# littlepure2333/GFlow

Measured on AMD Instinct MI355X. Metric: GFlow fit_video frames/sec (fwd+bwd+step) @60k Gaussians 480p, higher is better.
Workload: dtype f32

## Files before the change

gflow_amd/_lib.py:

```python
import ctypes
import os
import subprocess
import threading

import torch

_HERE = os.path.dirname(os.path.abspath(__file__))
_CSRC = os.path.join(_HERE, "csrc")
LIB_PATH = os.environ.get("GFLOW_HIP_LIB") or os.path.join(_HERE, "libgflow_hip.so")

_lock = threading.Lock()
_lib = None

c_void_p, c_int, c_float, c_size_t, c_int64 = ctypes.c_void_p, ctypes.c_int, ctypes.c_float, ctypes.c_size_t, ctypes.c_int64

MIN_VERSION = 308

_P = c_void_p
SIGNATURES = {
    "gfl_version": (c_int, []),
    "gfl_constants": (c_int, [_P]),
    "gfl_constants_n": (c_int, [_P, c_int]),
    "gfl_ewa_on_mfma": (c_int, []),
    "gfl_status_string": (ctypes.c_char_p, [c_int]),
    "gfl_last_hip_error": (c_int, []),
    "gfl_reduce_workspace_bytes": (c_size_t, [c_int]),
    "gfl_project_point_fwd": (c_int, [_P, _P, _P, c_int, c_int, c_int, c_float, c_float, _P, _P, _P]),
    "gfl_project_point_bwd": (c_int, [_P, _P, _P, _P, _P, _P, c_int, _P, _P, _P, c_size_t, _P]),
    "gfl_cov3d_fwd": (c_int, [_P, _P, _P, c_int, _P, _P]),
    "gfl_cov3d_bwd": (c_int, [_P, _P, _P, _P, c_int, _P, _P, _P]),
    "gfl_ewa_fwd": (c_int, [_P, _P, _P, _P, _P, _P, c_int, c_int, c_int, _P, _P, _P, _P]),
    "gfl_ewa_bwd": (c_int, [_P, _P, _P, _P, _P, _P, c_int, c_int, c_int, _P, _P, _P, _P, c_size_t, _P]),
    "gfl_bin_workspace_bytes": (c_size_t, [c_int, c_int, c_int, c_int]),
    "gfl_bin_count": (c_int, [_P, _P, _P, c_int, c_int, c_int, _P, _P]),
    "gfl_bin_sort": (c_int, [_P, _P, _P, _P, c_int, c_int, c_int, _P, c_int, _P, _P, _P, _P, c_size_t, _P]),
    "gfl_blend_fwd": (c_int, [_P, _P, _P, _P, c_int, c_int, c_int, _P, _P, c_float, c_int, c_int, _P, _P, _P, _P]),
    "gfl_blend_bwd": (c_int, [_P, _P, _P, _P, c_int, c_int, c_int, _P, _P, c_float, c_int, c_int, _P, _P, _P, c_int,
                              _P, _P, _P, _P, c_int, _P]),
    "gfl_sh_fwd": (c_int, [_P, _P, _P, c_int, c_int, _P, _P]),
    "gfl_sh_bwd": (c_int, [_P, _P, _P, _P, c_int, c_int, _P, _P, _P]),
    "gfl_colormap_nonzero": (c_int, [_P, c_int, _P, _P, _P, c_size_t, _P]),
    "gfl_loss_workspace_bytes": (c_size_t, [c_int, c_int]),
    "gfl_loss_fwd_bwd": (c_int, [_P, _P, _P, _P, _P, c_float, c_float, c_int, c_int, _P, _P, _P, _P, c_size_t, _P]),
    "gfl_loss_fwd_bwd_partials": (c_int, [_P, _P, _P, _P, _P, c_float, c_float, c_int, c_int, _P, _P, _P, c_size_t, _P, _P, _P, _P, _P]),
    "gfl_loss_prepare_gt": (c_int, [_P, _P, c_int, c_int, _P, _P]),
    "gfl_loss_fwd_bwd_partials_cached": (c_int, [_P, _P, _P, _P, _P, c_float, c_float, c_int, c_int, _P, _P, _P, c_size_t, _P, _P, _P, _P, _P, _P]),
    "gfl_adam_step": (c_int, [_P, _P, _P, _P, c_int64, c_int, _P, c_float, c_float, c_float, c_float, _P, c_float, c_int, _P]),
    "gfl_step_increment": (c_int, [_P, _P]),
    "gfl_tile_sort_only": (c_int, [_P, c_int, c_int, _P, _P, _P, _P]),
    "gfl_tile_sort_ordered": (c_int, [_P, c_int, c_int, c_int, _P, _P, _P, _P]),
    "gfl_tile_sort_reserved": (c_int, [_P, _P, _P, _P, c_int, c_int, c_int, _P, _P, _P, _P]),
    "gfl_fit_workspace_bytes": (c_size_t, [c_int, c_int, c_int, c_int]),
    "gfl_fit_forward": (c_int, [_P, _P, _P]),
    "gfl_fit_backward_step": (c_int, [_P, _P, _P]),
    "gfl_fit_iteration": (c_int, [_P, _P, _P]),
    "gfl_fit_iterations": (c_int, [_P, _P, c_int, c_int, _P]),
    "gfl_fit_reserved_supported": (c_int, [_P, _P]),
    "gfl_fit_snapshot_stage": (c_int, [_P, _P, _P]),
    "gfl_fit_snapshot_workspace_bytes": (c_size_t, [c_int, c_int, c_int]),
    "gfl_fit_snapshot": (c_int, [_P, _P, _P, _P, _P, c_size_t, _P]),
    "gfl_fit_iteration_snapshot": (c_int, [_P, _P, _P, _P, _P]),
    "gfl_render_fwd": (c_int, [_P, _P, _P]),
    "gfl_render_bwd": (c_int, [_P, _P, _P, _P, _P, _P, _P, _P]),
    "gfl_fit_prepare_targets": (c_int, [_P, _P]),
    "gfl_fit_schedule_info": (c_int, [_P, _P, _P, _P, _P]),
    "gfl_fit_schedule_info_fwd": (c_int, [_P, _P, _P, _P, _P]),
    "gfl_selftest_reduce10": (c_int, [_P, _P, _P, _P]),
    "gfl_selftest_cov2d": (c_int, [_P, _P, c_int, _P, _P, _P]),
    "gfl_selftest_block_mask": (c_int, [_P, c_int, c_int, c_int, c_int, _P, _P, _P]),
    "gfl_concave_hull": (c_int, [_P, c_int, ctypes.c_double, ctypes.c_double, _P, c_int]),
    "gfl_scan_f64_workspace_bytes": (c_size_t, [c_int]),
    "gfl_scan_f64": (c_int, [_P, c_int, _P, _P, c_size_t, _P]),
    "gfl_track_anchor_workspace_bytes": (c_size_t, [c_int, c_int]),
    "gfl_track_anchor": (c_int, [_P, c_int, c_int, _P, c_int, _P, _P, _P, c_size_t, _P]),
    "gfl_track_frame": (c_int, [_P, c_int, _P, c_int, c_int, _P, c_int, c_int, _P, _P, c_int, c_int, c_int, c_float, _P, _P,
                                _P]),
    "gfl_seg_score": (c_int, [_P, _P, _P, c_int, c_int, c_int, c_int, _P, _P]),
    "gfl_recon_workspace_bytes": (c_size_t, [c_int, c_int]),
    "gfl_recon_frame": (c_int, [_P, _P, c_int, c_int, c_int, c_int, _P, _P, c_size_t, _P]),
    "gfl_abi_sizes": (c_int, [_P, _P]),
    "gfl_profile_enable": (c_int, [ctypes.c_uint]),
    "gfl_profile_read": (c_int, [_P, _P, c_int]),
}


def build(force=False, quiet=True):
    if force:
        subprocess.run(["make", "-C", _CSRC, "clean"], check=True, capture_output=quiet)
    res = subprocess.run(["make", "-C", _CSRC, "-j8"], capture_output=True, text=True)
    if res.returncode != 0:
        raise RuntimeError("building libgflow_hip.so failed:\n" + res.stdout + res.stderr)
    return LIB_PATH


def load():
    global _lib
    with _lock:
        if _lib is not None:
            return _lib
        if not os.path.exists(LIB_PATH):
            raise RuntimeError(
                f"{LIB_PATH} is missing: run `python -c 'import __graft_entry__ as g; g.build()'` "
                "(or `make -C gflow_amd/csrc`).  gflow_amd has no CPU fallback.")
        lib = ctypes.CDLL(LIB_PATH)
        for name, (res, args) in SIGNATURES.items():
            fn = getattr(lib, name)
            fn.restype = res
            fn.argtypes = args
        if lib.gfl_version() < MIN_VERSION:
            raise RuntimeError(f"{LIB_PATH} is version {lib.gfl_version()}, this binding needs >= {MIN_VERSION}: rebuild it "
                               "(make -C gflow_amd/csrc)")
        _lib = lib
        return lib


def check(rc, what=""):
    if rc != 0:
        lib = load()
        msg = lib.gfl_status_string(rc).decode()
        extra = f" (hipError {lib.gfl_last_hip_error()})" if rc == -3 else ""
        raise RuntimeError(f"libgflow_hip: {what}: {msg}{extra}")


def ptr(t):
    return None if t is None else ctypes.c_void_p(t.data_ptr())


def stream():
    return ctypes.c_void_p(torch.cuda.current_stream().cuda_stream)


def need_device(*tensors):
    for t in tensors:
        if t is not None and not t.is_cuda:
            raise RuntimeError("gflow_amd: tensors must be on a HIP (cuda) device; there is no CPU fallback")


def scratch(nbytes, device):
    return torch.empty(max(int(nbytes), 16), dtype=torch.uint8, device=device)


def scan_f64(x):
    need_device(x)
    x = x.reshape(-1).double().contiguous()
    out = torch.empty_like(x)
    n = x.numel()
    if n:
        lib = load()
        ws = scratch(lib.gfl_scan_f64_workspace_bytes(n), x.device)
        check(lib.gfl_scan_f64(ptr(x), n, ptr(out), ptr(ws), ws.numel(), stream()), "scan_f64")
    return out


def resolve_deterministic(deterministic):
    return torch.are_deterministic_algorithms_enabled() if deterministic is None else bool(deterministic)


_hip = None


def _hip_runtime():
    global _hip
    if _hip is None:
        _hip = ctypes.CDLL("libamdhip64.so")
        _hip.hipExtStreamCreateWithCUMask.restype = ctypes.c_int
        _hip.hipExtStreamCreateWithCUMask.argtypes = [ctypes.POINTER(ctypes.c_void_p), ctypes.c_uint32,
                                                      ctypes.POINTER(ctypes.c_uint32)]
    return _hip


def cu_partition(parts, device=None, cus=None):
    if cus is None:
        cus = torch.cuda.get_device_properties(device if device is not None else torch.cuda.current_device()).multi_processor_count
    xcds = 8
    per_xcd = cus // xcds
    n = per_xcd // int(parts)
    if n < 1:
        raise ValueError(f"cu_partition: {parts} shares of {per_xcd} CUs per XCD")
    out = []
    for p in range(int(parts)):
        words = [0] * ((cus + 31) // 32)
        for cu in range(p * n, (p + 1) * n):
            for x in range(xcds):
                i = cu * xcds + x
                words[i // 32] |= 1 << (i % 32)
        out.append((words, n * xcds))
    return out


def masked_stream(words, device=None):
    dev = torch.device("cuda", torch.cuda.current_device()) if device is None else torch.device(device)
    with torch.cuda.device(dev):
        arr = (ctypes.c_uint32 * len(words))(*words)
        h = ctypes.c_void_p()
        rc = _hip_runtime().hipExtStreamCreateWithCUMask(ctypes.byref(h), len(words), arr)
        if rc != 0:
            raise RuntimeError(f"hipExtStreamCreateWithCUMask failed: hipError {rc}")
    return torch.cuda.ExternalStream(h.value, device=dev)
```

gflow_amd/csrc/gfl_fit.hip:

```cpp
#include "gfl_fit.hpp"

using namespace gfl;

extern "C" {

static inline size_t up256(size_t v) { return (v + 255) / 256 * 256; }

size_t gfl_loss_workspace_bytes(int W, int H);

static inline int fit_nblk(int N) { return (N + BIN_BLOCK - 1) / BIN_BLOCK; }

static bool ewa_on_mfma() {
    static int v = -1;
    if (v < 0) {
        const char* e = getenv("GFL_EWA_MFMA");
        v = (e && e[0] == '1') ? 1 : 0;
    }
    return v == 1;
}

int gfl_ewa_on_mfma(void) { return ewa_on_mfma() ? 1 : 0; }

static int fwd_split_min() {
    static int v = -1;
    if (v < 0) {
        const char* e = getenv("GFL_FWD_SPLIT_MIN");
        v = e ? atoi(e) : FWD_SPLIT_MIN;
    }
    return v;
}

static int device_cus() {
    static int cus = 0;
    if (!cus) {
        int dev = 0;
        if (hipGetDevice(&dev) != hipSuccess ||
            hipDeviceGetAttribute(&cus, hipDeviceAttributeMultiprocessorCount, dev) != hipSuccess || cus <= 0)
            cus = 256;
    }
    return cus;
}
static int blend_queues(const gfl_fit_state* st) {
    int cus = (st && st->cu_count > 0) ? (st->cu_count / 8) * 8 : device_cus();
    if (cus <= 0) cus = 8;
    if (st && st->cu_count > 0) return cus < SCHED_MAX_QUEUES ? cus : SCHED_MAX_QUEUES;
    return cus < 64 ? 64 : (cus < SCHED_MAX_QUEUES ? cus : SCHED_MAX_QUEUES);
}

static int blend_grid(const gfl_fit_state* st, int T, int max_per_cu = BLEND_WG_PER_CU) {
    const int nq = blend_queues(st);
    int per = (T + nq - 1) / nq + 1;
    if (per > max_per_cu) per = max_per_cu;
    return nq * per;
}


size_t gfl_fit_workspace_bytes(int cap, int K_cap, int W, int H) {
    if (cap < 0 || K_cap < 0 || W <= 0 || H <= 0) return 0;
    const size_t T = (size_t)((W + GFL_TILE - 1) / GFL_TILE) * ((H + GFL_TILE - 1) / GFL_TILE);
    return up256((size_t)fit_nblk(cap > 0 ? cap : 1) * T * sizeof(int32_t))
           + up256((size_t)K_cap * sizeof(unsigned long long))
           + up256((size_t)reduce_rows(cap > 0 ? cap : 1) * 12 * sizeof(float))
           + up256(T * sizeof(int32_t))
           + up256(((size_t)(cap > 0 ? cap : 1) * SLOT_MAX + (size_t)K_cap) * PG * sizeof(float))
           + up256((size_t)(cap > 0 ? cap : 1) * sizeof(int32_t))
           + 256
           + up256(4 * T * sizeof(int32_t))
           + up256((size_t)SCHED_MAX_QUEUES * sched_queue_capacity((int)T, 64) * sizeof(int32_t))
           + 2 * up256(2 * SCHED_MAX_QUEUES * sizeof(int32_t))
           + up256((size_t)SCHED_MAX_QUEUES * (HEAVY_PARTS - 1) * 5 * 256 * sizeof(float))
           + up256(4 * T * sizeof(int32_t)) + up256(T * sizeof(int32_t))
           + up256((size_t)SCHED_MAX_QUEUES * sched_queue_capacity((int)T, 64) * sizeof(int32_t))
           + up256(2 * SCHED_MAX_QUEUES * sizeof(int32_t))
           + up256(gfl_loss_workspace_bytes(W, H)) + 256
           + up256((size_t)6 * W * H * sizeof(float))
           + up256((size_t)2 * fit_nblk(cap > 0 ? cap : 1) * sizeof(int32_t))
           + up256((T * 4 + SORT_ORDER_TRAILER) * sizeof(int32_t))
           + up256((T * 4 + SORT_ORDER_TRAILER) * sizeof(int32_t))
           + up256(T * sizeof(int4)) + up256(T * sizeof(int32_t));
}


static FitWs carve(const gfl_fit_state* st) {
    const size_t T = (size_t)((st->W + GFL_TILE - 1) / GFL_TILE) * ((st->H + GFL_TILE - 1) / GFL_TILE);
    char* p = (char*)st->workspace;
    FitWs w;
    w.hist = (int32_t*)p;
    p += up256((size_t)fit_nblk(st->cap > 0 ? st->cap : 1) * T * sizeof(int32_t));
    w.keys = (unsigned long long*)p;
    p += up256((size_t)st->K_cap * sizeof(unsigned long long));
    w.partial = (float*)p;
    p += up256((size_t)reduce_rows(st->cap > 0 ? st->cap : 1) * 12 * sizeof(float));
    w.tile_counts = (int32_t*)p;
    p += up256(T * sizeof(int32_t));
    w.pair_grad = (float*)p;
    w.wide_base = (long long)(st->cap > 0 ? st->cap : 1) * SLOT_MAX;
    p += up256(((size_t)(st->cap > 0 ? st->cap : 1) * SLOT_MAX + (size_t)st->K_cap) * PG * sizeof(float));
    w.wide_off = (int32_t*)p;
    p += up256((size_t)(st->cap > 0 ? st->cap : 1) * sizeof(int32_t));
    w.pool_counter = (int32_t*)p;
    w.stamp = w.pool_counter + 56;
    w.snap_mm = (unsigned*)(w.pool_counter + 58);
    w.sched_valid = w.pool_counter + 16;
    w.regions_valid = w.pool_counter + 32;
    w.extent = w.pool_counter + 40;
    w.extent_next = w.pool_counter + 48;
    p += 256;
    w.sched.work = (int32_t*)p;
    p += up256(4 * T * sizeof(int32_t));
    w.sched.list = (int32_t*)p;
    p += up256((size_t)SCHED_MAX_QUEUES * sched_queue_capacity((int)T, 64) * sizeof(int32_t));
    w.sched.count = (int32_t*)p;
    p += up256(2 * SCHED_MAX_QUEUES * sizeof(int32_t));
    w.sched.counters = (int32_t*)p;
    p += up256(2 * SCHED_MAX_QUEUES * sizeof(int32_t));
    w.ckpt = (float*)p;
    p += up256((size_t)SCHED_MAX_QUEUES * (HEAVY_PARTS - 1) * 5 * 256 * sizeof(float));
    w.sched.nq = blend_queues(st);
    w.sched.cap_q = (int)(((size_t)SCHED_MAX_QUEUES * sched_queue_capacity((int)T, 64)) / w.sched.nq);
    w.sched.split_min = 0;
    w.sched.xcd = 1;
    w.sched.det = (st->flags & GFL_FIT_DETERMINISTIC) ? 1 : 0;
    w.sched_fwd = w.sched;
    w.sched_fwd.work = (int32_t*)p;
    p += up256(4 * T * sizeof(int32_t));
    w.sched_fwd.list = (int32_t*)p;
    p += up256((size_t)SCHED_MAX_QUEUES * sched_queue_capacity((int)T, 64) * sizeof(int32_t));
    w.sched_fwd.count = (int32_t*)p;
    p += up256(2 * SCHED_MAX_QUEUES * sizeof(int32_t));
    w.sched.first_slot = (int32_t*)p;
    p += up256(T * sizeof(int32_t));
    w.sched_fwd.first_slot = nullptr;
    w.sched_fwd.split_min = fwd_split_min();
    w.loss_ws = p;
    w.loss_ws_bytes = up256(gfl_loss_workspace_bytes(st->W, st->H));
    w.gt_stats = (float*)((char*)p + w.loss_ws_bytes + 256);
    w.scale_cnt = (int32_t*)((char*)w.gt_stats + up256((size_t)6 * st->W * st->H * sizeof(float)));
    w.sort_order = (int4*)((char*)w.scale_cnt + up256((size_t)2 * fit_nblk(st->cap > 0 ? st->cap : 1) * sizeof(int32_t)));
    w.sort_order_next = (int4*)((char*)w.sort_order + up256((T * 4 + SORT_ORDER_TRAILER) * sizeof(int32_t)));
    w.region = (int4*)((char*)w.sort_order_next + up256((T * 4 + SORT_ORDER_TRAILER) * sizeof(int32_t)));
    w.fill = (int32_t*)((char*)w.region + up256(T * sizeof(int4)));
    return w;
}

static bool next_sched_ok(const FitWs& w, int T) {
    return w.sched.xcd && T <= SCHED_PLAN_TILES && w.sched.nq % 8 == 0 && w.sched.nq / 8 <= 64 && w.sched.nq <= REDUCE_BLOCK;
}
static int next_sched_blocks(const FitWs& w, int T) { return next_sched_ok(w, T) ? 2 : 0; }
static size_t next_sched_lds(const FitWs& w, int T) { return next_sched_ok(w, T) ? sched_dyn_lds(T) : 0; }
static NextSched next_sched(const FitWs& w, int rows, int T) {
    NextSched ns;
    ns.rows = rows;
    ns.T = T;
    ns.tile_counts = w.tile_counts;
    ns.bwd = w.sched;
    ns.fwd = w.sched_fwd;
    ns.valid = w.sched_valid;
    ns.reserve = 0;
    ns.order_next = nullptr; ns.ro = ReserveOut{}; ns.regions_valid = nullptr; ns.pool_counter = nullptr;
    ns.pull_counters = nullptr; ns.n_pull = 0;
    return ns;
}

static bool reserved_enabled() {
    static int v = -1;
    if (v < 0) {
        const char* e = getenv("GFL_RESERVED");
        v = (e && e[0] == '0') ? 0 : 1;
    }
    return v == 1;
}
static bool fit_reserved_ok(const FitWs& w, int T) {
    return reserved_enabled() && next_sched_ok(w, T) && T <= 4096 && (2 * (size_t)T + 64) * sizeof(int32_t) <= 57 * 1024;
}
static NextSched next_sched_reserving(const gfl_fit_state* st, const FitWs& w, int rows, int T) {
    NextSched ns = next_sched(w, rows, T);
    if (!fit_reserved_ok(w, T)) return ns;
    ns.reserve = 1;
    ns.order_next = w.sort_order_next;
    ns.ro.region = w.region; ns.ro.fill = w.fill; ns.ro.extent_next = w.extent_next; ns.ro.total = st->tile_offsets + T;
    ns.ro.K_cap = st->K_cap;
    ns.regions_valid = w.regions_valid;
    ns.pool_counter = w.pool_counter;
    ns.pull_counters = w.sched.counters; ns.n_pull = 2 * w.sched.nq;
    return ns;
}

static int fit_check(const gfl_fit_state* st, const gfl_fit_hyper* hp) {
    if (!st || !hp) return GFL_ERR_INVALID;
    if (st->N < 0 || st->N > st->cap || st->W <= 0 || st->H <= 0 || st->K_cap < 0) return GFL_ERR_INVALID;
    if (st->flags & ~GFL_FIT_DETERMINISTIC) return GFL_ERR_INVALID;
    if (!st->params || !st->rec || !st->pose || !st->intr || !st->extr || !st->render || !st->final_T ||
        !st->n_contrib || !st->tile_offsets || !st->ids || !st->tile_range || !st->overflow || !st->workspace)
        return GFL_ERR_INVALID;
    if (st->workspace_bytes < gfl_fit_workspace_bytes(st->cap, st->K_cap, st->W, st->H)) return GFL_ERR_WORKSPACE;
    return GFL_OK;
}


static PreArgs pre_args(const gfl_fit_state* st, const gfl_fit_hyper* hp, const FitWs& w, int gx, int gy, int op_mode) {
    PreArgs a;
    a.intr = st->intr; a.pose = st->pose;
    a.N = st->N; a.W = st->W; a.H = st->H;
    a.nearest = hp->nearest; a.extent = hp->extent;
    a.gx = gx; a.gy = gy;
    a.rec = st->rec; a.wide_off = w.wide_off; a.hist_g = w.hist; a.extr_out = st->extr; a.overflow = st->overflow;
    a.pool_counter = w.pool_counter; a.pool_cap = st->K_cap;
    a.op_mode = op_mode;
    a.scale_rows_mode = (!op_mode && hp->lambda_scale != 0.f) ? (hp->freeze_all_splats ? 2 : 1) : 0;
    a.scale_cnt = w.scale_cnt;
    return a;
}

static int fit_forward_impl(const gfl_fit_state* st, const gfl_fit_hyper* hp, gfl_stream_t stream, int op_mode, int reserved = 0,
                            const float* snap_lut = nullptr, uint8_t* snap_u8 = nullptr) {
    int rc = fit_check(st, hp);
    if (rc) return rc;
    hipStream_t s = (hipStream_t)stream;
    const int gx = (st->W + GFL_TILE - 1) / GFL_TILE, gy = (st->H + GFL_TILE - 1) / GFL_TILE, T = gx * gy;
    const FitWs w = carve(st);
    const int nblk = fit_nblk(st->N > 0 ? st->N : 1);
    if ((size_t)T * sizeof(int32_t) > 57 * 1024) return GFL_ERR_INVALID;
    const PreArgs pa = pre_args(st, hp, w, gx, gy, op_mode);
    if (reserved) {
        if (op_mode || !fit_reserved_ok(w, T)) return GFL_ERR_INVALID;
        {
            StageScope p(ST_PREPROCESS, s);
            BinArgs b;
            b.region = w.region; b.fill = w.fill; b.keys = w.keys; b.K_cap = st->K_cap;
            b.regions_valid = w.regions_valid; b.extent_next = w.extent_next; b.extent = w.extent;
            b.pull_counters = w.sched.counters; b.n_pull = 2 * w.sched.nq;
            launch_preprocess_bin(st->params, pa, st->row_flags, b, nblk, ewa_on_mfma(), s);
        }
        {
            StageScope p(ST_TILE_SORT, s);
            rc = gfl_tile_sort_reserved((const int32_t*)w.sort_order_next, w.fill, w.tile_counts, st->overflow + 2, st->W, st->H,
                                        st->K_cap, w.keys, st->ids, st->tile_range, stream);
        }
        if (rc) return rc;
    } else {
        {
            StageScope p(ST_PREPROCESS, s);
            launch_preprocess_fwd(st->params, pa, st->row_flags, nblk, ewa_on_mfma(), s);
        }
        {
            StageScope p(ST_COLSCAN, s);
            launch_colscan(w, nblk, T, st->overflow, s);
        }
        const bool ordered = T <= 8 * BIN_BLOCK;
        {
            StageScope p(ST_SCATTER, s);
            launch_scatter(st, w, nblk, gx, gy, ordered, s);
        }
        {
            StageScope p(ST_TILE_SORT, s);
            if (ordered)
                rc = gfl_tile_sort_ordered((const int32_t*)w.sort_order, st->W, st->H, st->K_cap, w.keys, st->ids, st->tile_range,
                                           stream);
            else
                rc = gfl_tile_sort_only(st->tile_offsets, gx * gy, st->K_cap, w.keys, st->ids, st->tile_range, stream);
        }
        if (rc) return rc;
    }
    {
        StageScope p(ST_BLEND_FWD, s);
        const TileQueue q = {w.sched_fwd.list, w.sched_fwd.count, w.sched.counters, w.sched.nq, w.sched.cap_q};
        if (snap_u8) {
            rc = check(hipMemsetAsync(w.snap_mm, 0, 2 * sizeof(unsigned), s));
            if (rc) return rc;
            if (st->N > 0) launch_rec_depth_range(st->rec, st->N, w.snap_mm, s);
            launch_blend_fwd(st, hp->bg, gx, blend_grid(st, T, FWD_WG_PER_CU), st->render, st->final_T, st->n_contrib, q, w, 2,
                             w.snap_mm, snap_lut, fwd_split_min(), s, snap_u8);
            launch_center_blend(st, hp->bg, gx, T, nullptr, snap_u8 + (size_t)2 * st->W * st->H * 3, s);
        }
        const bool foot = st->foot_flags && !(hp->bg > 0.f) && st->N > 0;
        if (foot && !st->keep) return GFL_ERR_INVALID;
        const bool foot_inside = foot && !snap_u8;
        if (!snap_u8)
            launch_blend_fwd(st, hp->bg, gx, blend_grid(st, T, FWD_WG_PER_CU), st->render, st->final_T, st->n_contrib, q, w,
                             foot_inside ? 3 : 0, nullptr, nullptr, fwd_split_min(), s);
        if (st->foot_flags) {
            if (!st->keep) return GFL_ERR_INVALID;
            if (foot && !foot_inside) launch_footprint(st, gx, T, s);
        }
    }
    return check_launch();
}

int gfl_fit_forward(const gfl_fit_state* st, const gfl_fit_hyper* hp, gfl_stream_t stream) {
    return fit_forward_impl(st, hp, stream, 0);
}

size_t gfl_fit_snapshot_workspace_bytes(int N, int W, int H) {
    if (N < 0 || W <= 0 || H <= 0) return 0;
    return 256 + up256(2 * SCHED_MAX_QUEUES * sizeof(int32_t)) + 2 * up256((size_t)4 * W * H * sizeof(float)) +
           up256((size_t)W * H * sizeof(float)) + up256((size_t)W * H * sizeof(int32_t));
}

int gfl_fit_snapshot(const gfl_fit_state* st, const gfl_fit_hyper* hp, const float* lut, uint8_t* out_u8, void* workspace,
                     size_t workspace_bytes, gfl_stream_t stream) {
    int rc = fit_check(st, hp);
    if (rc) return rc;
    if (!lut || !out_u8 || !workspace) return GFL_ERR_INVALID;
    if (workspace_bytes < gfl_fit_snapshot_workspace_bytes(st->N, st->W, st->H)) return GFL_ERR_WORKSPACE;
    hipStream_t s = (hipStream_t)stream;
    const int gx = (st->W + GFL_TILE - 1) / GFL_TILE, gy = (st->H + GFL_TILE - 1) / GFL_TILE, T = gx * gy;
    const int P = st->W * st->H;
    const FitWs w = carve(st);
    char* p = (char*)workspace;
    unsigned* mm = (unsigned*)p;                 p += 256;
    int32_t* pull = (int32_t*)p;                 p += up256(2 * SCHED_MAX_QUEUES * sizeof(int32_t));
    const size_t head_bytes = (size_t)(p - (char*)workspace);
    float* img_dc = (float*)p;                   p += up256((size_t)4 * P * sizeof(float));
    float* img_c = (float*)p;                    p += up256((size_t)4 * P * sizeof(float));
    float* fT = (float*)p;                       p += up256((size_t)P * sizeof(float));
    int32_t* nc = (int32_t*)p;
    rc = check(hipMemsetAsync(workspace, 0, head_bytes, s));
    if (rc) return rc;
    if (st->N > 0) launch_rec_depth_range(st->rec, st->N, mm, s);
    launch_center_blend(st, hp->bg, gx, T, img_c, nullptr, s);
    {
        const TileQueue q = {w.sched_fwd.list, w.sched_fwd.count, pull, w.sched.nq, w.sched.cap_q};
        launch_blend_fwd(st, hp->bg, gx, blend_grid(st, T, FWD_WG_PER_CU), img_dc, fT, nc, q, w, 1, mm, lut, fwd_split_min(), s);
    }
    launch_snapshot_u8(st->render, img_dc, img_c, P, out_u8, s);
    return check_launch();
}

int gfl_fit_snapshot_stage(const gfl_fit_state* src, const gfl_fit_state* dst, gfl_stream_t stream) {
    if (!src || !dst || !src->workspace || !dst->workspace || !src->rec || !dst->rec || !src->ids || !dst->ids ||
        !src->tile_range || !dst->tile_range || !src->render || !dst->render || !src->tile_offsets)
        return GFL_ERR_INVALID;
    if (src->W != dst->W || src->H != dst->H || src->N != dst->N || dst->N > dst->cap || src->N > src->cap)
        return GFL_ERR_INVALID;
    if (src->workspace_bytes < gfl_fit_workspace_bytes(src->cap, src->K_cap, src->W, src->H) ||
        dst->workspace_bytes < gfl_fit_workspace_bytes(dst->cap, dst->K_cap, dst->W, dst->H))
        return GFL_ERR_WORKSPACE;
    const int gx = (src->W + GFL_TILE - 1) / GFL_TILE, gy = (src->H + GFL_TILE - 1) / GFL_TILE, T = gx * gy;
    const size_t P = (size_t)src->W * src->H;
    const FitWs a = carve(src), b = carve(dst);
    if (a.sched_fwd.nq != b.sched_fwd.nq || a.sched_fwd.cap_q != b.sched_fwd.cap_q) return GFL_ERR_INVALID;
    StageCopy c;
    c.k_ptr = a.extent;
    c.ids_cap = (unsigned)min(src->K_cap, dst->K_cap);
    c.seg[0] = {(const uint32_t*)src->ids, (uint32_t*)dst->ids, 0u};
    c.seg[1] = {(const uint32_t*)src->rec, (uint32_t*)dst->rec, (unsigned)((size_t)src->N * REC)};
    c.seg[2] = {(const uint32_t*)src->tile_range, (uint32_t*)dst->tile_range, (unsigned)(2 * T)};
    c.seg[3] = {(const uint32_t*)src->render, (uint32_t*)dst->render, (unsigned)(3 * P)};
    c.seg[4] = {(const uint32_t*)a.sched_fwd.list, (uint32_t*)b.sched_fwd.list,
                (unsigned)((size_t)a.sched_fwd.nq * a.sched_fwd.cap_q)};
    c.seg[5] = {(const uint32_t*)a.sched_fwd.count, (uint32_t*)b.sched_fwd.count, (unsigned)a.sched_fwd.nq};
    c.seg[6] = {(const uint32_t*)a.sched.first_slot, (uint32_t*)b.sched.first_slot, (unsigned)T};
    launch_snapshot_stage(c, (hipStream_t)stream);
    return check_launch();
}

int gfl_render_fwd(const gfl_fit_state* st, const gfl_fit_hyper* hp, gfl_stream_t stream) {
    if (st && st->foot_flags) return GFL_ERR_INVALID;
    if (st && (st->flags & GFL_FIT_DETERMINISTIC)) {
        const int rc = fit_check(st, hp);
        if (rc) return rc;
        const int T = ((st->W + GFL_TILE - 1) / GFL_TILE) * ((st->H + GFL_TILE - 1) / GFL_TILE);
        const FitWs w = carve(st);
        hipStream_t s = (hipStream_t)stream;
        if (check(hipMemsetAsync(w.sched.work, 0, 4 * (size_t)T * sizeof(int32_t), s)) ||
            check(hipMemsetAsync(w.sched_fwd.work, 0, 4 * (size_t)T * sizeof(int32_t), s)) ||
            check(hipMemsetAsync(w.sched_valid, 0, sizeof(int32_t), s)))
            return GFL_ERR_HIP;
    }
    return fit_forward_impl(st, hp, stream, 1);
}

int gfl_render_bwd(const gfl_fit_state* st, const gfl_fit_hyper* hp, const float* d_render, const float* d_uv,
                   const float* d_depth, float* d_params, float* d_extr, gfl_stream_t stream) {
    int rc = fit_check(st, hp);
    if (rc) return rc;
    if (!d_render || !d_params || !d_extr) return GFL_ERR_INVALID;
    hipStream_t s = (hipStream_t)stream;
    const int gx = (st->W + GFL_TILE - 1) / GFL_TILE, gy = (st->H + GFL_TILE - 1) / GFL_TILE, T = gx * gy;
    const FitWs w = carve(st);
    {
        StageScope p(ST_BLEND_BWD, s);
        const TileQueue q = {w.sched.list, w.sched.count, w.sched.counters + w.sched.nq, w.sched.nq, w.sched.cap_q};
        launch_blend_bwd(st, hp->bg, gx, gy, blend_grid(st, T), 10, d_render, q, w, LossTail{}, s);
    }
    {
        StageScope p(ST_PRE_BWD_ADAM, s);
        const NextSched ns = next_sched(w, reduce_rows(st->N > 0 ? st->N : 1), T);
        launch_splat_bwd_op(st, w, gx, gy, ns, next_sched_blocks(w, T), next_sched_lds(w, T), d_uv, d_depth, d_params, d_extr, s);
    }
    return check_launch();
}

int gfl_fit_backward_step(const gfl_fit_state* st, const gfl_fit_hyper* hp, gfl_stream_t stream) {
    int rc = fit_check(st, hp);
    if (rc) return rc;
    if (!st->adam_m || !st->adam_v || !st->pose_m || !st->pose_v || !st->depth_ab || !st->depth_ab_m ||
        !st->depth_ab_v || !st->step || !st->gt_rgb || !st->d_render || !st->err_px || !st->sums || !st->d_extr)
        return GFL_ERR_INVALID;
    hipStream_t s = (hipStream_t)stream;
    const int gx = (st->W + GFL_TILE - 1) / GFL_TILE, gy = (st->H + GFL_TILE - 1) / GFL_TILE, T = gx * gy;
    const FitWs w = carve(st);
    const float *p_ssim = nullptr, *p_grad = nullptr;
    int n_ssim = 0, n_grad = 0;
    {
        StageScope p(ST_LOSS, s);
        const float* gt_stats = (st->gt_cached && !st->foot_flags) ? w.gt_stats : nullptr;
        rc = gfl_loss_fwd_bwd_partials_cached(st->render, st->gt_rgb, st->gt_depth, st->keep, st->depth_ab,
                                              hp->lambda_rgb, hp->lambda_depth, st->W, st->H, st->d_render,
                                              st->err_px, w.loss_ws, w.loss_ws_bytes, gt_stats, &p_ssim, &n_ssim,
                                              &p_grad, &n_grad, stream);
    }
    if (rc) return rc;
    AdamCfg ac = {hp->lr, hp->beta1, hp->beta2, hp->eps, hp->lr_end_factor, hp->total_iters};
    AdamCfg ac_cam = ac;
    ac_cam.lr = hp->lr_camera;
    const bool frozen = hp->step_camera != 2 && (hp->step_camera == 0 || hp->lr_camera == 0.f);
    LossTail lt = {};
    if (frozen) {
        lt.enabled = 1;
        lt.p_ssim = p_ssim; lt.n_ssim = n_ssim; lt.p_grad = p_grad; lt.n_grad = n_grad;
        lt.depth_ab = st->depth_ab; lt.ab_m = st->depth_ab_m; lt.ab_v = st->depth_ab_v;
        lt.sums = st->sums; lt.ac_ab = ac; lt.step_affine = hp->step_camera != 0;
        lt.d_step = st->step; lt.d_extr_out = st->d_extr; lt.overflow = st->overflow;
    }
    {
        StageScope p(ST_BLEND_BWD, s);
        const TileQueue q = {w.sched.list, w.sched.count, w.sched.counters + w.sched.nq, w.sched.nq, w.sched.cap_q};
        const int sums = hp->freeze_all_splats ? 6 : (hp->freeze_rgb ? 7 : 10);
        launch_blend_bwd(st, hp->bg, gx, gy, blend_grid(st, T), sums, st->d_render, q, w, lt, s);
    }
    const int rows = reduce_rows(st->N > 0 ? st->N : 1);
    RegCfg rcfg;
    rcfg.lambda_scale = hp->lambda_scale;
    rcfg.scale_blocks = 2 * fit_nblk(st->N > 0 ? st->N : 1);
    rcfg.lambda_var = st->N > 0 ? hp->lambda_var / (float)st->N : 0.f;
    rcfg.lambda_flow = hp->lambda_flow;
    rcfg.lambda_still = hp->lambda_still;
    rcfg.freeze_rgb = hp->freeze_rgb;
    rcfg.freeze_all = hp->freeze_all_splats;
    rcfg.no_pose_grad = frozen ? 1 : 0;
    {
        StageScope p(ST_PRE_BWD_ADAM, s);
        const NextSched ns = next_sched_reserving(st, w, rows, T);
        launch_splat_bwd_adam(st, w, gx, gy, rcfg, ac, ns, next_sched_blocks(w, T) + ns.reserve, next_sched_lds(w, T), s);
    }
    if (!frozen) {
        StageScope p(ST_CAMERA, s);
        launch_camera_adam(st, w, rows, p_ssim, n_ssim, p_grad, n_grad, ac_cam, ac, hp->step_camera != 0, s);
    }
    return check_launch();
}

int gfl_fit_iterations(const gfl_fit_state* st, const gfl_fit_hyper* hp, int count, int flags, gfl_stream_t stream) {
    if (count < 1 || (flags & ~GFL_ITER_RESERVED)) return GFL_ERR_INVALID;
    int rc = fit_check(st, hp);
    if (rc) return rc;
    const int T = ((st->W + GFL_TILE - 1) / GFL_TILE) * ((st->H + GFL_TILE - 1) / GFL_TILE);
    const FitWs w = carve(st);
    const bool res_ok = fit_reserved_ok(w, T) && st->N > 0;
    if ((flags & GFL_ITER_RESERVED) && !res_ok) return GFL_ERR_INVALID;
    for (int j = 0; j < count; ++j) {
        const int reserved = res_ok && (j > 0 || (flags & GFL_ITER_RESERVED)) ? 1 : 0;
        rc = fit_forward_impl(st, hp, stream, 0, reserved);
        if (rc) return rc;
        rc = gfl_fit_backward_step(st, hp, stream);
        if (rc) return rc;
    }
    return GFL_OK;
}

int gfl_fit_iteration_snapshot(const gfl_fit_state* st, const gfl_fit_hyper* hp, const float* lut, uint8_t* out_u8,
                               gfl_stream_t stream) {
    if (!lut || !out_u8) return GFL_ERR_INVALID;
    int rc = fit_forward_impl(st, hp, stream, 0, 0, lut, out_u8);
    if (rc) return rc;
    return gfl_fit_backward_step(st, hp, stream);
}

int gfl_fit_reserved_supported(const gfl_fit_state* st, const gfl_fit_hyper* hp) {
    if (fit_check(st, hp) || st->N <= 0) return 0;
    const int T = ((st->W + GFL_TILE - 1) / GFL_TILE) * ((st->H + GFL_TILE - 1) / GFL_TILE);
    return fit_reserved_ok(carve(st), T) ? 1 : 0;
}

int gfl_fit_prepare_targets(const gfl_fit_state* st, gfl_stream_t stream) {
    if (!st || st->W <= 0 || st->H <= 0 || !st->gt_rgb || !st->workspace) return GFL_ERR_INVALID;
    if (st->workspace_bytes < gfl_fit_workspace_bytes(st->cap, st->K_cap, st->W, st->H)) return GFL_ERR_WORKSPACE;
    const FitWs w = carve(st);
    return gfl_loss_prepare_gt(st->gt_rgb, st->keep, st->W, st->H, w.gt_stats, stream);
}

int gfl_fit_schedule_info(const gfl_fit_state* st, int* n_queues, int* queue_capacity, const int32_t** d_lists,
                          const int32_t** d_counts) {
    if (!st || !n_queues || !queue_capacity || !d_lists || !d_counts || !st->workspace) return GFL_ERR_INVALID;
    if (st->workspace_bytes < gfl_fit_workspace_bytes(st->cap, st->K_cap, st->W, st->H)) return GFL_ERR_WORKSPACE;
    const FitWs w = carve(st);
    *n_queues = w.sched.nq;
    *queue_capacity = w.sched.cap_q;
    *d_lists = w.sched.list;
    *d_counts = w.sched.count;
    return GFL_OK;
}

int gfl_fit_schedule_info_fwd(const gfl_fit_state* st, int* n_queues, int* queue_capacity, const int32_t** d_lists,
                              const int32_t** d_counts) {
    if (!st || !n_queues || !queue_capacity || !d_lists || !d_counts || !st->workspace) return GFL_ERR_INVALID;
    if (st->workspace_bytes < gfl_fit_workspace_bytes(st->cap, st->K_cap, st->W, st->H)) return GFL_ERR_WORKSPACE;
    const FitWs w = carve(st);
    *n_queues = w.sched_fwd.nq;
    *queue_capacity = w.sched_fwd.cap_q;
    *d_lists = w.sched_fwd.list;
    *d_counts = w.sched_fwd.count;
    return GFL_OK;
}

int gfl_fit_iteration(const gfl_fit_state* st, const gfl_fit_hyper* hp, gfl_stream_t stream) {
    int rc = gfl_fit_forward(st, hp, stream);
    if (rc) return rc;
    return gfl_fit_backward_step(st, hp, stream);
}

#ifdef GFL_TRACE
int gfl_debug_read_fwd_trace(long long* out, int n_tiles) { return read_fwd_trace(out, n_tiles); }
int gfl_debug_read_fwd_trace2(long long* out, int n_values) { return read_fwd_trace2(out, n_values); }
int gfl_debug_read_phase_trace(long long* out, int n_values) {
    const int rc = read_phase_trace_bin(out, n_values);
    return rc ? rc : read_phase_trace_splat(out, n_values);
}
int gfl_debug_read_bwd_trace(long long* out, int n_tiles) { return read_bwd_trace(out, n_tiles); }
#endif

}
```

gflow_amd/csrc/gfl_fit.hpp:

```cpp
#pragma once
#include "gfl_math.hpp"
#include "gfl_profile.hpp"
#include "gfl_sched.hpp"

#include <stdlib.h>

namespace gfl {

constexpr int BIN_BLOCK = 512;
#ifndef GFL_RBIN_BLOCK
#define GFL_RBIN_BLOCK 512
#endif
constexpr int RBIN_BLOCK = GFL_RBIN_BLOCK;
static_assert(RBIN_BLOCK == 256 || RBIN_BLOCK == 512, "two scale-row partials per 512 splats (PreArgs.scale_cnt)");
#ifndef GFL_WIDE_TILES
#define GFL_WIDE_TILES 16
#endif
constexpr int WIDE_TILES = GFL_WIDE_TILES;
constexpr int ROW = 16;
constexpr int REC = 12;
#ifndef GFL_PG_STRIDE
#define GFL_PG_STRIDE 12
#endif
constexpr int PG = GFL_PG_STRIDE;

__device__ __forceinline__ float sigmoidf_(float x) { return 1.0f / (1.0f + __expf(-x)); }

#ifdef GFL_TRACE
constexpr int PHASE_WAVES = 4096;
static __device__ long long g_phase_trace[4 * PHASE_WAVES * 8];
#define GFL_PHASE(kernel, slot)                                                                                      \
    do {                                                                                                             \
        const int w_ = blockIdx.x * (blockDim.x >> 6) + (threadIdx.x >> 6);                                          \
        if ((threadIdx.x & 63) == 0 && w_ < PHASE_WAVES) g_phase_trace[((kernel) * PHASE_WAVES + w_) * 8 + (slot)] = wall_clock64(); \
    } while (0)
#else
#define GFL_PHASE(kernel, slot) do {} while (0)
#endif

__device__ __forceinline__ Cam cam_from_pose(const float* __restrict__ intr, const float* __restrict__ pose) {
#pragma clang fp contract(off)
    Cam c;
    c.fx = intr[0]; c.fy = intr[1]; c.cx = intr[2]; c.cy = intr[3];
    float x = pose[0], y = pose[1], z = pose[2], w = pose[3];
    const float inv = 1.0f / sqrtf(x * x + y * y + z * z + w * w);
    x *= inv; y *= inv; z *= inv; w *= inv;
    c.r00 = 1.f - 2.f * (y * y + z * z); c.r01 = 2.f * (x * y - w * z); c.r02 = 2.f * (x * z + w * y);
    c.r10 = 2.f * (x * y + w * z); c.r11 = 1.f - 2.f * (x * x + z * z); c.r12 = 2.f * (y * z - w * x);
    c.r20 = 2.f * (x * z - w * y); c.r21 = 2.f * (y * z + w * x); c.r22 = 1.f - 2.f * (x * x + y * y);
    c.t0 = pose[4]; c.t1 = pose[5]; c.t2 = pose[6];
    return c;
}

struct Splat {
    float x, y, z;
    float s[3], raw_s[3];
    float q[4], raw_q[4], qn;
    float o, c[3];
};

__device__ __forceinline__ Splat splat_from_row(const float4& a, const float4& b, const float4& c, const float4& d,
                                                bool activated = false) {
#pragma clang fp contract(off)
    Splat s;
    s.x = a.x; s.y = a.y; s.z = a.z;
    s.raw_s[0] = a.w; s.raw_s[1] = b.x; s.raw_s[2] = b.y;
    s.raw_q[0] = b.z; s.raw_q[1] = b.w; s.raw_q[2] = c.x; s.raw_q[3] = c.y;
    if (activated) {
#pragma unroll
        for (int k = 0; k < 3; ++k) s.s[k] = s.raw_s[k];
#pragma unroll
        for (int k = 0; k < 4; ++k) s.q[k] = s.raw_q[k];
        s.qn = 1.f;
        s.o = c.z;
        s.c[0] = c.w; s.c[1] = d.x; s.c[2] = d.y;
        return s;
    }
#pragma unroll
    for (int k = 0; k < 3; ++k) s.s[k] = fabsf(s.raw_s[k]);
    s.qn = fmaxf(sqrtf(s.raw_q[0] * s.raw_q[0] + s.raw_q[1] * s.raw_q[1] + s.raw_q[2] * s.raw_q[2] +
                       s.raw_q[3] * s.raw_q[3]), 1e-12f);
#pragma unroll
    for (int k = 0; k < 4; ++k) s.q[k] = s.raw_q[k] / s.qn;
    s.o = sigmoidf_(10.0f * c.z);
    s.c[0] = sigmoidf_(c.w); s.c[1] = sigmoidf_(d.x); s.c[2] = sigmoidf_(d.y);
    return s;
}

__device__ __forceinline__ float alpha_cutoff(float o, float lam) {
#pragma clang fp contract(off)
    if (o < GFL_ALPHA_MIN) return -1.0f;
    const float r = 255.0f * o;
    if (r < 1.05f) return 3.0e38f;
    return 2.0f * __logf(r) * lam * 1.002f + 0.01f;
}

__device__ __forceinline__ bool tile_hit2(float u, float v, float cutoff, int tx, int ty) {
#pragma clang fp contract(off)
    const float x_lo = (float)(tx * GFL_TILE), x_hi = x_lo + (float)(GFL_TILE - 1);
    const float y_lo = (float)(ty * GFL_TILE), y_hi = y_lo + (float)(GFL_TILE - 1);
    u = gridf(u); v = gridf(v);
    const float ddx = fmaxf(fmaxf(x_lo - u, u - x_hi), 0.f);
    const float ddy = fmaxf(fmaxf(y_lo - v, v - y_hi), 0.f);
    return ddx * ddx + ddy * ddy <= cutoff;
}

__device__ __forceinline__ bool scale_row(float u, float v, int W, int H, unsigned flags, int mode) {
    const bool within = u > 0.f && u < (float)(W - 1) && v > 0.f && v < (float)(H - 1);
    const bool labelled = flags & 2u, still = flags & 1u;
    return within && (!labelled || (mode == 2 ? still : !still));
}

struct PreArgs {
    const float* intr; const float* pose;
    int N, W, H;
    float nearest, extent;
    int gx, gy;
    float* rec; int32_t* wide_off; int32_t* hist_g; float* extr_out; int32_t* overflow;
    int32_t* pool_counter; int pool_cap; int op_mode;
    int scale_rows_mode; int32_t* scale_cnt;
};

struct PreOut { float u, v, cutoff, depth; int rad; };
struct BinArgs {
    const int4* region;
    int32_t* fill;
    unsigned long long* keys;
    int K_cap;
    int32_t* regions_valid;
    const int32_t* extent_next;
    int32_t* extent;
    int32_t* pull_counters; int n_pull;
};

__host__ __device__ __forceinline__ int region_cap(int c) { return c + (c >> 2) + 32; }
struct ReserveOut { int4* region; int32_t* fill; int32_t* extent_next; int32_t* total; int K_cap; };

constexpr int BLEND_WG_PER_CU = 8;
constexpr int FWD_WG_PER_CU = 5;
constexpr int FWD_UNITS = 4;
constexpr int FWD_SPLIT_MIN = 448;
constexpr int FB = 256;
#ifndef GFL_FWD_LONG_BATCH
#define GFL_FWD_LONG_BATCH 256
#endif
constexpr int FBL = GFL_FWD_LONG_BATCH;
constexpr int FBB = 192;
constexpr int FBB_DET = 64;

struct WgVote {
    int32_t* cnt;
    int base0, base1, round;
};
__device__ __forceinline__ WgVote wg_vote_init(int32_t* lds2) {
    WgVote v;
    v.cnt = lds2; v.base0 = 0; v.base1 = 0; v.round = 0;
    return v;
}
__device__ __forceinline__ bool wg_all(WgVote& v, bool pred, int waves) {
    const int r = v.round & 1;
    if (__all(pred) && (threadIdx.x & 63) == 0) atomicAdd(&v.cnt[r], 1);
    __syncthreads();
    const int now = v.cnt[r];
    const bool all = now - (r ? v.base1 : v.base0) == waves;
    if (r) v.base1 = now; else v.base0 = now;
    ++v.round;
    return all;
}

__device__ __forceinline__ void tile_xy(int tile, int gx, unsigned inv_gx, int& tx, int& ty) {
    ty = (int)__umulhi((unsigned)tile, inv_gx);
    tx = tile - ty * gx;
}

struct RecLDS {
    float4 p0, p1, p2;
};

__device__ __forceinline__ bool splat_alpha2(const float4& p0, const float4& p1, float fx, float fy, float& alpha,
                                             float& G) {
#pragma clang fp contract(off)
    const float dx = p0.x - fx, dy = p0.y - fy;
    const float q = __builtin_fmaf(p0.z * dx, dx, (p1.x * dy) * dy);
    const float power = __builtin_fmaf(-0.5f, q, -((p0.w * dx) * dy));
    G = __expf(fminf(power, 0.f));
    alpha = fminf(GFL_ALPHA_MAX, p1.y * G);
    return (power <= 0.f) & (alpha >= GFL_ALPHA_MIN);
}

__device__ __forceinline__ uint8_t img_u8(float v) {
    const float x = fminf(fmaxf(v, 0.f), 1.f) * 255.f;
    return (uint8_t)(x != x ? 0.f : x);
}

struct AdamCfg {
    float lr, b1, b2, eps, lr_end_factor;
    int total_iters;
};

__device__ __forceinline__ void adam_scalars(const AdamCfg& a, int e, float lr, float& step_size, float& inv_sqrt_bc2) {
    const float t = (float)(e + 1);
    if (a.total_iters > 0) lr *= 1.f + (a.lr_end_factor - 1.f) * (float)min(e, a.total_iters) / (float)a.total_iters;
    step_size = lr / (1.f - powf(a.b1, t));
    inv_sqrt_bc2 = 1.f / sqrtf(1.f - powf(a.b2, t));
}

__device__ __forceinline__ float adam_update(float p, float g, float& m, float& v, const AdamCfg& a, float step_size,
                                             float inv_sqrt_bc2) {
    m = fmaf(a.b1, m, (1.f - a.b1) * g);
    v = fmaf(a.b2, v, (1.f - a.b2) * g * g);
    const float denom = sqrtf(v) * inv_sqrt_bc2 + a.eps;
    return p - step_size * (m / denom);
}

struct LossTail {
    int enabled;
    const float* p_ssim; int n_ssim;
    const float* p_grad; int n_grad;
    float* depth_ab; float* ab_m; float* ab_v;
    float* sums;
    AdamCfg ac_ab;
    int step_affine;
    int32_t* d_step;
    float* d_extr_out;
    int32_t* overflow;
};

struct RegCfg {
    float lambda_scale;
    int scale_blocks;
    float lambda_var;
    float lambda_flow;
    float lambda_still;
    int freeze_rgb;
    int freeze_all;
    int no_pose_grad;
};

struct NextSched {
    int rows;
    int T;
    const int32_t* tile_counts;
    Sched bwd, fwd;
    int32_t* valid;
    int reserve;
    int4* order_next;
    ReserveOut ro;
    int32_t* regions_valid;
    int32_t* pool_counter;
    int32_t* pull_counters;
    int n_pull;
};

struct FitWs {
    int32_t* hist;
    unsigned long long* keys;
    float* partial;
    int32_t* tile_counts;
    float* pair_grad;
    int32_t* wide_off;
    long long wide_base;
    int32_t* stamp;
    unsigned* snap_mm;
    int32_t* pool_counter;
    int32_t* sched_valid;
    Sched sched;
    Sched sched_fwd;
    float* ckpt;
    void* loss_ws;
    size_t loss_ws_bytes;
    float* gt_stats;
    int32_t* scale_cnt;
    int4* sort_order;
    int4* sort_order_next;
    int4* region;
    int32_t* fill;
    int32_t* regions_valid;
    int32_t* extent;
    int32_t* extent_next;
};

inline size_t sched_dyn_lds(int T) {
    return (size_t)T * sizeof(int32_t) + (T <= SCHED_PLAN_TILES ? (size_t)SCHED_PLAN_TILES * sizeof(uint32_t) : 0);
}

struct StageSeg { const uint32_t* src; uint32_t* dst; unsigned n; };
struct StageCopy { StageSeg seg[7]; const int32_t* k_ptr; unsigned ids_cap; };

void launch_preprocess_fwd(const float* params, const PreArgs& a, const uint8_t* row_flags, int nblk, bool mfma, hipStream_t s);
void launch_preprocess_bin(const float* params, const PreArgs& a, const uint8_t* row_flags, const BinArgs& b, int nblk, bool mfma,
                           hipStream_t s);
void launch_colscan(const FitWs& w, int nblk, int T, int32_t* overflow, hipStream_t s);
void launch_scatter(const gfl_fit_state* st, const FitWs& w, int nblk, int gx, int gy, bool ordered, hipStream_t s);
inline unsigned inv_of(int gx) { return (unsigned)((((unsigned long long)1 << 32) + (unsigned)gx - 1) / (unsigned)gx); }
void launch_blend_fwd(const gfl_fit_state* st, float bg, int gx, int grid, float* out, float* final_T, int32_t* n_contrib,
                      const TileQueue& q, const FitWs& w, int mode, const unsigned* cmap_mm, const float* cmap_lut, int split_min,
                      hipStream_t s, uint8_t* snap_u8 = nullptr);
void launch_footprint(const gfl_fit_state* st, int gx, int T, hipStream_t s);
void launch_center_blend(const gfl_fit_state* st, float bg, int gx, int T, float* out, uint8_t* out_u8, hipStream_t s);
void launch_rec_depth_range(const float* rec, int N, unsigned* mm, hipStream_t s);
void launch_snapshot_u8(const float* a, const float* b, const float* c, int P, uint8_t* out, hipStream_t s);
void launch_snapshot_stage(const StageCopy& c, hipStream_t s);
void launch_blend_bwd(const gfl_fit_state* st, float bg, int gx, int gy, int grid, int sums, const float* d_out, const TileQueue& q,
                      const FitWs& w, const LossTail& lt, hipStream_t s);
void launch_splat_bwd_adam(const gfl_fit_state* st, const FitWs& w, int gx, int gy, const RegCfg& rc, const AdamCfg& ac,
                           const NextSched& ns, int extra, size_t lds, hipStream_t s);
void launch_splat_bwd_op(const gfl_fit_state* st, const FitWs& w, int gx, int gy, const NextSched& ns, int extra, size_t lds,
                         const float* d_uv, const float* d_depth, float* d_params, float* d_extr, hipStream_t s);
void launch_camera_adam(const gfl_fit_state* st, const FitWs& w, int rows, const float* p_ssim, int n_ssim, const float* p_grad,
                        int n_grad, const AdamCfg& ac_cam, const AdamCfg& ac_ab, int step_camera, hipStream_t s);
#ifdef GFL_TRACE
int read_phase_trace_bin(long long* out, int n_values);
int read_phase_trace_splat(long long* out, int n_values);
int read_fwd_trace(long long* out, int n_tiles);
int read_fwd_trace2(long long* out, int n_values);
int read_bwd_trace(long long* out, int n_tiles);
#endif

}
```

gflow_amd/csrc/gfl_fit_bwd.hip:

```cpp
#include "gfl_fit.hpp"

namespace gfl {

__device__ __forceinline__ void blend_bwd_terms(const float4& p0, const float4& p1, const float4& p2, float fx, float fy,
                                                bool valid, float alpha, float G, float g0, float g1, float g2, float g3,
                                                float& T, float& S, float (&v)[10]) {
    const float a_eff = valid ? alpha : 0.f;
    const float rom = __builtin_amdgcn_rcpf(1.f - a_eff);
    T = T * rom;
    const float h = fmaf(g0, p1.z, fmaf(g1, p1.w, fmaf(g2, p2.x, g3 * p2.y)));
    const float dalpha = valid ? fmaf(T, h, -(S * rom)) : 0.f;
    const float w = a_eff * T;
    S = fmaf(h, w, S);
    v[6] = w * g0; v[7] = w * g1; v[8] = w * g2; v[9] = w * g3;
    const float dx = p0.x - fx, dy = p0.y - fy;
    v[5] = G * dalpha;
    const float dpow = p1.y * v[5];
    const float mx = -dx * dpow, my = -dy * dpow;
    v[0] = mx;
    v[1] = my;
    v[2] = dx * mx;
    v[3] = dx * my;
    v[4] = dy * my;
}

#ifdef GFL_TRACE
__device__ long long g_bwd_trace[16384 * 8];
#endif
template <int B = 256>
__device__ void loss_tail(const LossTail& t) {
    constexpr int NV = 5;
    __shared__ float red[B / 64][NV];
    __shared__ float ge[NV];
    float ab[2] = {0.f, 0.f}, abm[2] = {0.f, 0.f}, abv[2] = {0.f, 0.f};
    int e_step = 0;
    if (threadIdx.x == 0) {
        e_step = *t.d_step;
#pragma unroll
        for (int k = 0; k < 2; ++k) { ab[k] = t.depth_ab[k]; abm[k] = t.ab_m[k]; abv[k] = t.ab_v[k]; }
    }
    float acc[NV] = {0.f, 0.f, 0.f, 0.f, 0.f};
    for (int r0 = threadIdx.x; r0 < t.n_ssim; r0 += 8 * B) {
        float v[8];
#pragma unroll
        for (int u = 0; u < 8; ++u) v[u] = (r0 + u * B < t.n_ssim) ? t.p_ssim[r0 + u * B] : 0.f;
#pragma unroll
        for (int u = 0; u < 8; ++u) acc[1] += v[u];
    }
    for (int r0 = threadIdx.x; r0 < t.n_grad; r0 += 4 * B) {
        float4 q[4];
#pragma unroll
        for (int u = 0; u < 4; ++u)
            q[u] = (r0 + u * B < t.n_grad) ? reinterpret_cast<const float4*>(t.p_grad)[r0 + u * B]
                                           : make_float4(0.f, 0.f, 0.f, 0.f);
#pragma unroll
        for (int u = 0; u < 4; ++u) { acc[0] += q[u].x; acc[2] += q[u].y; acc[3] += q[u].z; acc[4] += q[u].w; }
    }
    const int lane = threadIdx.x & 63, wid = threadIdx.x >> 6;
#pragma unroll
    for (int k = 0; k < NV; ++k) {
        const float s = wave_sum_to_lane63(acc[k]);
        if (lane == 63) red[wid][k] = s;
    }
    __syncthreads();
    if (threadIdx.x < NV) {
        float x = 0.f;
#pragma unroll
        for (int w = 0; w < B / 64; ++w) x += red[w][threadIdx.x];
        ge[threadIdx.x] = x;
        t.sums[threadIdx.x] = x;
    }
    if (threadIdx.x >= NV && threadIdx.x < NV + 3) t.sums[threadIdx.x] = 0.f;
    if (threadIdx.x >= 16 && threadIdx.x < 28) t.d_extr_out[threadIdx.x - 16] = 0.f;
    __syncthreads();
    if (threadIdx.x == 0) {
        if (t.overflow && (t.overflow[0] | t.overflow[2]) != 0) {
            t.overflow[1] += 1;
            return;
        }
        if (t.step_affine) {
            float ss, isb;
            adam_scalars(t.ac_ab, e_step, t.ac_ab.lr, ss, isb);
#pragma unroll
            for (int k = 0; k < 2; ++k) {
                t.depth_ab[k] = adam_update(ab[k], ge[3 + k], abm[k], abv[k], t.ac_ab, ss, isb);
                t.ab_m[k] = abm[k]; t.ab_v[k] = abv[k];
            }
        }
        *t.d_step = e_step + 1;
    }
}

template <int SUMS, bool DET = false>
__global__ void __launch_bounds__(256, 8) fused_blend_bwd_kernel(const float* __restrict__ rec,
                                                              const int32_t* __restrict__ ids,
                                                              const int32_t* __restrict__ tile_range, float bg, int W,
                                                              int H, int gx, const float* __restrict__ final_T,
                                                              const int32_t* __restrict__ n_contrib,
                                                              const float* __restrict__ d_out,
                                                              float* __restrict__ pair_grad, TileQueue queue,
                                                              int32_t* __restrict__ tile_work,
                                                              const float* __restrict__ ckpt,
                                                              const float* __restrict__ render, LossTail ltail, int gy,
                                                              const int32_t* __restrict__ wide_off, long long wide_base,
                                                              const int32_t* __restrict__ stamp_ptr) {
    if (ltail.enabled && blockIdx.x == gridDim.x - queue.nq) loss_tail(ltail);
    constexpr int NB = DET ? FBB_DET : FBB;
    constexpr int NACC = DET ? 4 : 1;
    static_assert(!DET || NACC * NB * REC == 3 * 4 * 256, "the deterministic rows are cleared with three float4 per lane");
    __shared__ RecLDS recs[NB];
    __shared__ int32_t s_gid[NB];
    __shared__ float acc[NACC][NB][REC];
    __shared__ unsigned char s_mask[NB];
    __shared__ int32_t s_max_last;
    __shared__ int32_t s_ticket;
    __shared__ int32_t s_simd[4];
    const int tid = threadIdx.x, wave = tid >> 6, lane = tid & 63;
    const int comp_few = SUMS == 6 ? reduce_scatter6_component(lane) : reduce_scatter7_component(lane);
    const int comp = SUMS == 10 ? reduce_scatter10_component(lane) : (comp_few == SUMS - 1 ? 9 : comp_few);
    unsigned hw_id;
    asm volatile("s_getreg_b32 %0, hwreg(HW_REG_HW_ID)" : "=s"(hw_id));
    const int simd = (hw_id >> 4) & 3;
    if (lane == 0) s_simd[wave] = simd;
    __syncthreads();
    const bool simd_ok = ((1 << s_simd[0]) | (1 << s_simd[1]) | (1 << s_simd[2]) | (1 << s_simd[3])) == 15;
  for (bool first = true;; first = false) {
    const TileItem item = next_item(queue, &s_ticket, first, HEAVY_PARTS, gridDim.x);
    const int tile = item.tile;
    if (tile < 0) break;
    const unsigned plan = item.plan;
    const bool plan_ok = simd_ok && ((1 << (plan & 3)) | (1 << ((plan >> 2) & 3)) | (1 << ((plan >> 4) & 3)) | (1 << ((plan >> 6) & 3))) == 15;
    const int blk = plan_ok ? (int)((plan >> (2 * simd)) & 3u) : wave;
    const int tx = tile % gx, ty = tile / gx;
    const int px = tx * GFL_TILE + (blk & 1) * 8 + (lane & 7);
    const int py = ty * GFL_TILE + (blk >> 1) * 8 + (lane >> 3);
    const bool inside = px < W && py < H;
    const float fx = pixf(px), fy = pixf(py);
    const int start = tile_range[2 * tile], end = tile_range[2 * tile + 1];
    const int total = end - start;
    const int parts = item.part >= 0 ? heavy_parts(total) : 1;
    if (item.part >= parts) continue;
    const int seg = heavy_seg(total, parts);
    const bool last_part = item.part < 0 || item.part == parts - 1;
    int units = 0;
#ifdef GFL_TRACE
    const long long trace_t0 = wall_clock64();
    int trace_lanes = 0;
#endif

    float g0 = 0.f, g1 = 0.f, g2 = 0.f, g3 = 0.f, T = 1.f, S = 0.f;
    int last = 0;
    if (inside) {
        const size_t pix = (size_t)py * W + px, plane = (size_t)H * W;
        last = n_contrib[pix];
        g0 = d_out[pix]; g1 = d_out[plane + pix]; g2 = d_out[2 * plane + pix]; g3 = d_out[3 * plane + pix];
        if (last_part) {
            T = final_T[pix];
            S = T * bg * (g0 + g1 + g2 + g3);
        } else {
            const float* ck = ckpt + ((size_t)item.queue * (HEAVY_PARTS - 1) + item.part) * 5 * 256 + blk * 64 + lane;
            T = ck[0];
            S = g0 * (render[pix] - ck[256]) + g1 * (render[plane + pix] - ck[512]) +
                g2 * (render[2 * plane + pix] - ck[768]) + g3 * (render[3 * plane + pix] - ck[1024]);
        }
    }
    if (tid == 0) s_max_last = 0;
    __syncthreads();
    const unsigned long long alive0 = __ballot(inside);
    const int px0w = tx * GFL_TILE + (blk & 1) * 8, py0w = ty * GFL_TILE + (blk >> 1) * 8;
    int wave_last = last;
#pragma unroll
    for (int off = 32; off >= 1; off >>= 1) wave_last = max(wave_last, __shfl_xor(wave_last, off));
    if (lane == 0) atomicMax(&s_max_last, wave_last);
    __syncthreads();
    const int depth_n = min(total, (int)s_max_last);
    const float4 zero4 = make_float4(0.f, 0.f, 0.f, 0.f);

    const int lo = item.part > 0 ? item.part * seg : 0;
    const int hi = last_part ? depth_n : min((item.part + 1) * seg, depth_n);

    const int stamp = *stamp_ptr;
    for (int r0 = 0; r0 < hi - lo; r0 += NB) {
        const int pos_t = tid < NB ? hi - 1 - r0 - tid : -1;
        __syncthreads();
        if (pos_t >= lo) {
            const int g = ids[start + pos_t];
            const float4* r4 = reinterpret_cast<const float4*>(rec + (size_t)g * REC);
            const float4 p0 = r4[0], p1 = r4[1], p2 = r4[2];
            recs[tid].p0 = p0; recs[tid].p1 = p1; recs[tid].p2 = p2;
            s_gid[tid] = g;
            s_mask[tid] = (unsigned char)block_mask(p0, p1, p2.z, tx * GFL_TILE, ty * GFL_TILE);
        }
        if constexpr (DET) {
            float4* az = reinterpret_cast<float4*>(&acc[0][0][0]);
            az[tid] = zero4; az[tid + 256] = zero4; az[tid + 512] = zero4;
        } else if (tid < NB) {
            float4* az = reinterpret_cast<float4*>(&acc[0][tid][0]);
            az[0] = zero4; az[1] = zero4; az[2] = zero4;
        }
        __syncthreads();
        const int cnt = min(NB, hi - lo - r0);
        for (int c0 = 0; c0 < cnt; c0 += 64) {
            const int slot = c0 + lane;
            const int spos = hi - 1 - r0 - slot;
            bool hit = slot < cnt && spos < wave_last && ((s_mask[slot] >> blk) & 1);
            {
                const unsigned long long alive = __ballot(last > hi - 1 - r0 - c0 - 63);
                if (alive != alive0 && alive != 0ull) {
                    unsigned long long a = alive | (alive >> 32);
                    a |= a >> 16;
                    a |= a >> 8;
                    const unsigned cols = (unsigned)a & 0xffu;
                    const int xl = __builtin_ctz(cols), xh = 31 - __builtin_clz(cols);
                    const int yl = (int)__builtin_ctzll(alive) >> 3, yh = (63 - (int)__builtin_clzll(alive)) >> 3;
                    if (hit) {
                        const BlockTest t = block_test(recs[slot].p0, recs[slot].p1, recs[slot].p2.z);
                        hit = box_hit(t, (float)(px0w + xl), (float)(px0w + xh), (float)(py0w + yl), (float)(py0w + yh));
                    }
                }
            }
            unsigned long long bits = __ballot(hit);
            while (bits) {
                const int j = c0 + (int)__builtin_ctzll(bits);
                bits &= bits - 1;
                const int pos = hi - 1 - r0 - j;
                const float4 p0 = recs[j].p0, p1 = recs[j].p1, p2 = recs[j].p2;
                float alpha, G;
                const bool valid = splat_alpha2(p0, p1, fx, fy, alpha, G) && (pos < last);
                if (__ballot(valid) == 0ull) continue;
#ifdef GFL_TRACE
                trace_lanes += __popcll(__ballot(valid));
#endif
                ++units;
                float v[10];
                blend_bwd_terms(p0, p1, p2, fx, fy, valid, alpha, G, g0, g1, g2, g3, T, S, v);
                float mine;
                if (SUMS == 6) {
                    const float v6[6] = {v[0], v[1], v[2], v[3], v[4], v[9]};
                    mine = wave_reduce_scatter6(v6, lane);
                } else if (SUMS == 7) {
                    const float v7[7] = {v[0], v[1], v[2], v[3], v[4], v[5], v[9]};
                    mine = wave_reduce_scatter7(v7, lane);
                } else {
                    mine = wave_reduce_scatter10(v, lane);
                }
                if constexpr (DET) {
                    if (comp >= 0) acc[blk][j][comp] = mine;
                } else {
                    if (comp >= 0) atomicAdd(&acc[0][j][comp], mine);
                }
            }
        }
        __syncthreads();
        if (pos_t >= lo) {
            const int g = s_gid[tid];
            const float4 p0 = recs[tid].p0;
            int x0, x1, y0, y1;
            tile_rect(p0.x, p0.y, __float_as_int(recs[tid].p2.w), gx, gy, x0, x1, y0, y1);
            const int nx = x1 - x0, j = (ty - y0) * nx + (tx - x0);
            long long row = (long long)g * SLOT_MAX + j;
            if (nx * (y1 - y0) > SLOT_MAX) {
                const int off = wide_off[g];
                row = off >= 0 ? wide_base + off + j : -1;
            }
            if (row >= 0) {
                float4* o = reinterpret_cast<float4*>(pair_grad + (size_t)row * PG);
                if constexpr (DET) {
                    float4 s[3];
#pragma unroll
                    for (int k = 0; k < 3; ++k) {
                        const float4 b0 = reinterpret_cast<const float4*>(&acc[0][tid][0])[k];
                        const float4 b1 = reinterpret_cast<const float4*>(&acc[1][tid][0])[k];
                        const float4 b2 = reinterpret_cast<const float4*>(&acc[2][tid][0])[k];
                        const float4 b3 = reinterpret_cast<const float4*>(&acc[3][tid][0])[k];
                        s[k] = make_float4(((b0.x + b1.x) + b2.x) + b3.x, ((b0.y + b1.y) + b2.y) + b3.y,
                                           ((b0.z + b1.z) + b2.z) + b3.z, ((b0.w + b1.w) + b2.w) + b3.w);
                    }
                    o[0] = s[0]; o[1] = s[1];
                    o[2] = make_float4(s[2].x, s[2].y, __int_as_float(stamp), 0.f);
                } else {
                    const float4* a4 = reinterpret_cast<const float4*>(&acc[0][tid][0]);
                    o[0] = a4[0]; o[1] = a4[1];
                    o[2] = make_float4(a4[2].x, a4[2].y, __int_as_float(stamp), 0.f);
                }
            }
        }
    }
    if (lane == 0) atomicAdd(&tile_work[4 * tile + blk], units + 1);
#ifdef GFL_TRACE
    if (lane == 0 && tile < 2048) {
        unsigned hw, xcc;
        asm volatile("s_getreg_b32 %0, hwreg(HW_REG_HW_ID)" : "=s"(hw));
        asm volatile("s_getreg_b32 %0, hwreg(HW_REG_XCC_ID)" : "=s"(xcc));
        long long* tr = g_bwd_trace + (size_t)(tile + (last_part ? 0 : 2048 * (1 + item.part))) * 8;
        if (wave == 0) {
            tr[0] = trace_t0; tr[1] = wall_clock64();
            tr[2] = ((long long)total << 32) | (unsigned)depth_n;
            tr[3] = ((long long)(xcc & 15) << 32) | hw;
        }
        tr[4 + wave] = ((long long)(trace_lanes | ((hw >> 4) & 3) << 28) << 32) | (unsigned)units;
    }
#endif
  }
}

void launch_blend_bwd(const gfl_fit_state* st, float bg, int gx, int gy, int grid, int sums, const float* d_out, const TileQueue& q,
                      const FitWs& w, const LossTail& lt, hipStream_t s) {
    auto kern = sums == 6 ? fused_blend_bwd_kernel<6> : (sums == 7 ? fused_blend_bwd_kernel<7> : fused_blend_bwd_kernel<10>);
    if (st->flags & GFL_FIT_DETERMINISTIC)
        kern = sums == 6 ? fused_blend_bwd_kernel<6, true>
                         : (sums == 7 ? fused_blend_bwd_kernel<7, true> : fused_blend_bwd_kernel<10, true>);
    kern<<<grid, 256, 0, s>>>(st->rec, st->ids, st->tile_range, bg, st->W, st->H, gx, st->final_T, st->n_contrib, d_out, w.pair_grad,
                              q, w.sched.work, w.ckpt, st->render, lt, gy, w.wide_off, w.wide_base, w.stamp);
}

#ifdef GFL_TRACE
int read_bwd_trace(long long* out, int n_tiles) {
    return (int)hipMemcpyFromSymbol(out, HIP_SYMBOL(g_bwd_trace), (size_t)n_tiles * 8 * sizeof(long long));
}
#endif

}
```

gflow_amd/csrc/gfl_ssim.hip:

```cpp
#include "gfl_common.hpp"

#include <math.h>

namespace gfl {

constexpr int SW = 11;
constexpr int SR = SW / 2;
constexpr int ST = 16;
constexpr int SI = ST + 2 * SR;
constexpr int SP = 48;
constexpr int HP = 24;
constexpr float SSIM_C1 = 0.01f * 0.01f;
constexpr float SSIM_C2 = 0.03f * 0.03f;

struct Win { float w[SW]; };

__device__ __forceinline__ void load16(const float* __restrict__ row, float (&v)[16]) {
    const float4* p = reinterpret_cast<const float4*>(row);
    const float4 a = p[0], b = p[1], c = p[2], d = p[3];
    v[0] = a.x; v[1] = a.y; v[2] = a.z; v[3] = a.w; v[4] = b.x; v[5] = b.y; v[6] = b.z; v[7] = b.w;
    v[8] = c.x; v[9] = c.y; v[10] = c.z; v[11] = c.w; v[12] = d.x; v[13] = d.y; v[14] = d.z; v[15] = d.w;
}

__device__ __forceinline__ float ld_f32(const float* __restrict__ base, unsigned byte_off) {
    return *reinterpret_cast<const float*>(reinterpret_cast<const char*>(base) + byte_off);
}
__device__ __forceinline__ unsigned pixel_index(int y, int W, int x) { return __umul24((unsigned)y, (unsigned)W) + (unsigned)x; }
__device__ __forceinline__ void st_f32(float* __restrict__ base, unsigned byte_off, float v) {
    *reinterpret_cast<float*>(reinterpret_cast<char*>(base) + byte_off) = v;
}

__device__ __forceinline__ void load12(const float* __restrict__ row, float (&v)[12]) {
    const float4* p = reinterpret_cast<const float4*>(row);
    const float4 a = p[0], b = p[1], c = p[2];
    v[0] = a.x; v[1] = a.y; v[2] = a.z; v[3] = a.w; v[4] = b.x; v[5] = b.y; v[6] = b.z; v[7] = b.w;
    v[8] = c.x; v[9] = c.y; v[10] = c.z; v[11] = c.w;
}

typedef float v2f __attribute__((ext_vector_type(2)));

template <int MODE, bool KEEP>
__global__ void __launch_bounds__(256) ssim_stats_kernel(const float* __restrict__ render,
                                                         const float* __restrict__ gt_rgb,
                                                         const uint8_t* __restrict__ keep, int W, int H, int gx,
                                                         int gy, Win win, float scale ,
                                                         float* __restrict__ dmaps, float* __restrict__ partial,
                                                         float* __restrict__ gt_stats) {
    constexpr int APITCH = 48, ROWS = SI + 1;
    __shared__ __attribute__((aligned(16))) v2f s_a[ROWS][APITCH];
    __shared__ __attribute__((aligned(16))) v2f s_b[MODE == 0 ? ROWS : 1][APITCH];
    __shared__ __attribute__((aligned(16))) float s_x_y[MODE == 2 ? 1 : ROWS][APITCH];
    __shared__ __attribute__((aligned(16))) v2f h_a[SI][ST];
    __shared__ __attribute__((aligned(16))) v2f h_b[MODE == 0 ? SI : 1][ST];
    __shared__ __attribute__((aligned(16))) float h_xy[MODE == 2 ? 1 : SI][ST];
    const int lb = __builtin_amdgcn_readfirstlane(xcd_logical_block(blockIdx.x, gx * gy * 3));
    const int c = lb % 3, tile = lb / 3;
    const int bx = tile % gx, by = tile / gx;
    const int x0 = bx * ST - SR, y0 = by * ST - SR;
    const int tid = threadIdx.x;
    const unsigned plane_b = (unsigned)H * (unsigned)W * 4u;
    float mu2_own = 0.f, e22_own = 0.f;
    if (MODE == 1) {
        const int opx = bx * ST + (tid & 15), opy = by * ST + (tid >> 4);
        if (opx < W && opy < H) {
            const unsigned ob = (pixel_index(opy, W, opx)) * 4u + 2u * c * plane_b;
            mu2_own = ld_f32(gt_stats, ob);
            e22_own = ld_f32(gt_stats, ob + plane_b);
        }
    }
    constexpr int NS = 4;
    const int sq = tid & 31, srg = tid >> 5;
    const int sx = x0 + sq;
    const bool in_x = sq < SI && sx >= 0 && sx < W;
    const unsigned c_plane_b = (unsigned)c * plane_b;
    float xs[NS], ys[NS];
    int kb[NS];
#pragma unroll
    for (int j = 0; j < NS; ++j) {
        const int y = y0 + srg + 8 * j;
        const bool in = in_x && (srg + 8 * j) < SI && (unsigned)y < (unsigned)H;
        const unsigned pix = in ? pixel_index(y, W, sx) : 0u;
        const unsigned pix4 = pix << 2;
        xs[j] = MODE == 2 ? 0.f : ld_f32(render, pix4 + c_plane_b);
        ys[j] = ld_f32(gt_rgb, pix4 + (pix4 << 1) + 4u * c);
        kb[j] = KEEP ? (int)keep[pix] : 1;
    }
#pragma unroll
    for (int j = 0; j < NS; ++j) {
        const int y = y0 + srg + 8 * j;
        const bool k = in_x && (srg + 8 * j) < SI && (unsigned)y < (unsigned)H && kb[j] != 0;
        const float xv = k ? xs[j] : 0.f, yv = k ? ys[j] : 0.f;
        const int r = min(srg + 8 * j, SI);
        if (MODE == 0) {
            s_a[r][sq] = (v2f){xv, yv};
            s_b[r][sq] = (v2f){xv * xv, yv * yv};
        } else if (MODE == 1) {
            s_a[r][sq] = (v2f){xv, xv * xv};
        } else {
            s_a[r][sq] = (v2f){yv, yv * yv};
        }
        if (MODE != 2) s_x_y[r][sq] = xv * yv;
    }
    __syncthreads();
    if (tid < SI * 8) {
        const int r = tid >> 3, q = (tid & 7) * 2;
        v2f A[12], B[12];
        float X[12];
#pragma unroll
        for (int k = 0; k < 12; k += 2) {
            const float4 t = *reinterpret_cast<const float4*>(&s_a[r][q + k]);
            A[k] = (v2f){t.x, t.y};
            A[k + 1] = (v2f){t.z, t.w};
            if (MODE == 0) {
                const float4 u = *reinterpret_cast<const float4*>(&s_b[r][q + k]);
                B[k] = (v2f){u.x, u.y};
                B[k + 1] = (v2f){u.z, u.w};
            }
            if (MODE != 2) {
                const float2 u = *reinterpret_cast<const float2*>(&s_x_y[r][q + k]);
                X[k] = u.x;
                X[k + 1] = u.y;
            }
        }
        v2f a_a[2] = {{0.f, 0.f}, {0.f, 0.f}}, a_b[2] = {{0.f, 0.f}, {0.f, 0.f}};
        float a_xy[2] = {0.f, 0.f};
#pragma unroll
        for (int k = 0; k < SW; ++k) {
            const float w = win.w[k];
            const v2f w2 = {w, w};
#pragma unroll
            for (int o = 0; o < 2; ++o) {
                a_a[o] = __builtin_elementwise_fma(w2, A[o + k], a_a[o]);
                if (MODE == 0) a_b[o] = __builtin_elementwise_fma(w2, B[o + k], a_b[o]);
                if (MODE != 2) a_xy[o] = fmaf(w, X[o + k], a_xy[o]);
            }
        }
        *reinterpret_cast<float4*>(&h_a[r][q]) = make_float4(a_a[0].x, a_a[0].y, a_a[1].x, a_a[1].y);
        if (MODE == 0) *reinterpret_cast<float4*>(&h_b[r][q]) = make_float4(a_b[0].x, a_b[0].y, a_b[1].x, a_b[1].y);
        if (MODE != 2) *reinterpret_cast<float2*>(&h_xy[r][q]) = make_float2(a_xy[0], a_xy[1]);
    }
    __syncthreads();
    const int lx = tid & 15, ly = tid >> 4;
    const int px = bx * ST + lx, py = by * ST + ly;
    float sval = 0.f;
    if (px < W && py < H) {
        v2f fa = {0.f, 0.f}, fb = {0.f, 0.f};
        float e12 = 0.f;
#pragma unroll
        for (int k = 0; k < SW; ++k) {
            const float w = win.w[k];
            const v2f w2 = {w, w};
            fa = __builtin_elementwise_fma(w2, h_a[ly + k][lx], fa);
            if (MODE == 0) fb = __builtin_elementwise_fma(w2, h_b[ly + k][lx], fb);
            if (MODE != 2) e12 = fmaf(w, h_xy[ly + k][lx], e12);
        }
        const unsigned pb = (pixel_index(py, W, px)) * 4u;
        if (MODE == 2) {
            st_f32(gt_stats, pb + 2u * c * plane_b, fa.x);
            st_f32(gt_stats, pb + (2u * c + 1u) * plane_b, fa.y);
            return;
        }
        float mu1, mu2, e11, e22;
        if (MODE == 0) {
            mu1 = fa.x; mu2 = fa.y; e11 = fb.x; e22 = fb.y;
        } else {
            mu1 = fa.x; e11 = fa.y;
            mu2 = mu2_own;
            e22 = e22_own;
        }
        const float mu1s = mu1 * mu1, mu2s = mu2 * mu2, mu12 = mu1 * mu2;
        const float s1 = e11 - mu1s, s2 = e22 - mu2s, s12 = e12 - mu12;
        const float A1 = 2.f * mu12 + SSIM_C1, A2 = 2.f * s12 + SSIM_C2;
        const float B1 = mu1s + mu2s + SSIM_C1, B2 = s1 + s2 + SSIM_C2;
        const float r1 = __builtin_amdgcn_rcpf(B1), r2 = __builtin_amdgcn_rcpf(B2);
        const float inv = r1 * r2;
        sval = A1 * A2 * inv;
        const float d_e11 = -sval * r2;
        const float d_e12 = 2.f * A1 * inv;
        const float d_mu1 = 2.f * mu2 * (A2 - A1) * inv - 2.f * mu1 * sval * (r1 - r2);
        const unsigned mb = pb + 3u * c * plane_b;
        st_f32(dmaps, mb, scale * d_mu1);
        st_f32(dmaps, mb + plane_b, scale * d_e11);
        st_f32(dmaps, mb + 2u * plane_b, scale * d_e12);
    }
    if (MODE == 2) return;
    float v[1] = {sval};
    const int bid = c * gx * gy + tile;
    __shared__ float red[4];
    const float s = wave_sum_to_lane63(v[0]);
    if ((tid & 63) == 63) red[tid >> 6] = s;
    __syncthreads();
    if (tid == 0) partial[bid] = red[0] + red[1] + red[2] + red[3];
}

template <bool KEEP>
__global__ void __launch_bounds__(256) loss_grad_kernel(
    const float* __restrict__ render, const float* __restrict__ gt_rgb, const float* __restrict__ gt_depth,
    const uint8_t* __restrict__ keep, const float* __restrict__ depth_ab, const float* __restrict__ dmaps, int W, int H,
    int gx, int gy, Win win, float mse_scale , float depth_scale ,
    float* __restrict__ d_render, float* __restrict__ err_px, float* __restrict__ partial) {
    __shared__ __attribute__((aligned(16))) float sm[3][SI + 1][SP];
    __shared__ __attribute__((aligned(16))) float hz[3][SI][HP];
    const int tid = threadIdx.x;
    const size_t plane = (size_t)H * W;
    const unsigned plane_b = (unsigned)H * (unsigned)W * 4u;
    const int lb = __builtin_amdgcn_readfirstlane(xcd_logical_block(blockIdx.x, gx * gy * 4));
    const int ch = lb & 3, tile = lb >> 2;
    const int bx = tile % gx, by = tile / gx;
    if (ch == 3) {
        const int lx = tid & 15, ly = tid >> 4;
        const int px = bx * ST + lx, py = by * ST + ly;
        float v[4] = {0.f, 0.f, 0.f, 0.f};
        if (px < W && py < H) {
            const size_t pix = (size_t)py * W + px;
            const int kb = KEEP ? (int)keep[pix] : 1;
            float rr[3], gg[3];
#pragma unroll
            for (int c = 0; c < 3; ++c) {
                rr[c] = render[c * plane + pix];
                gg[c] = gt_rgb[pix * 3 + c];
            }
            const bool with_depth = depth_scale != 0.f;
            const float D = with_depth ? render[3 * plane + pix] : 0.f;
            const float gt = with_depth ? gt_depth[pix] : 0.f;
            const bool k = kb != 0;
            float e = 0.f;
#pragma unroll
            for (int c = 0; c < 3; ++c) {
                const float d = k ? (rr[c] - gg[c]) : 0.f;
                e = fmaf(d, d, e);
            }
            e *= (1.f / 3.f);
            err_px[pix] = e;
            v[0] = e;
            float gD = 0.f;
            if (with_depth) {
                const float a = depth_ab[0], b = depth_ab[1];
                const float d = fmaf(a, D, b);
                const float diff = d - gt, sum = d + gt;
                if (k) {
                    v[1] = diff * diff / sum;
                    const float dl = depth_scale * diff * (d + 3.f * gt) / (sum * sum);
                    gD = dl * a;
                    v[2] = dl * D;
                    v[3] = dl;
                }
            }
            d_render[3 * plane + pix] = gD;
        }
        __shared__ float red[4][4];
#pragma unroll
        for (int q = 0; q < 4; ++q) {
            const float s = wave_sum_to_lane63(v[q]);
            if ((tid & 63) == 63) red[tid >> 6][q] = s;
        }
        __syncthreads();
        if (tid < 4) partial[(size_t)tile * 4 + tid] = red[0][tid] + red[1][tid] + red[2][tid] + red[3][tid];
        return;
    }
    const int x0 = bx * ST - SR, y0 = by * ST - SR;
    float own_x[2] = {0.f, 0.f}, own_y[2] = {0.f, 0.f};
    int own_kb[2] = {0, 0};
    if (tid < 128) {
        const int r0 = (tid >> 4) * 2, col = tid & 15;
        const int px = bx * ST + col;
#pragma unroll
        for (int o = 0; o < 2; ++o) {
            const int py = by * ST + r0 + o;
            if (px < W && py < H) {
                const unsigned pix = pixel_index(py, W, px);
                own_kb[o] = KEEP ? (int)keep[pix] : 1;
                own_x[o] = ld_f32(render, pix * 4u + ch * plane_b);
                own_y[o] = ld_f32(gt_rgb, pix * 12u + ch * 4u);
            }
        }
    }
    constexpr int NG = 4;
    const int sq = tid & 31, srg = tid >> 5;
    const int sx = x0 + sq;
    const bool in_x = sq < SI && sx >= 0 && sx < W;
    const unsigned map_b = 3u * ch * plane_b;
    float dm[NG][3];
#pragma unroll
    for (int j = 0; j < NG; ++j) {
        const int y = y0 + srg + 8 * j;
        const bool in = in_x && (srg + 8 * j) < SI && (unsigned)y < (unsigned)H;
        const unsigned pb = (in ? (pixel_index(y, W, sx)) << 2 : 0u) + map_b;
        dm[j][0] = ld_f32(dmaps, pb);
        dm[j][1] = ld_f32(dmaps, pb + plane_b);
        dm[j][2] = ld_f32(dmaps, pb + 2u * plane_b);
    }
#pragma unroll
    for (int j = 0; j < NG; ++j) {
        const int y = y0 + srg + 8 * j;
        const bool in = in_x && (srg + 8 * j) < SI && (unsigned)y < (unsigned)H;
        const int r = min(srg + 8 * j, SI);
        sm[0][r][sq] = in ? dm[j][0] : 0.f;
        sm[1][r][sq] = in ? dm[j][1] : 0.f;
        sm[2][r][sq] = in ? dm[j][2] : 0.f;
    }
    __syncthreads();
    for (int it = tid; it < 3 * SI * 4; it += 256) {
        const int m = it / (SI * 4), rem = it - m * (SI * 4);
        const int r = rem >> 2, q = (rem & 3) * 4;
        float X[16];
        load16(&sm[m][r][q], X);
        float a[4] = {0.f, 0.f, 0.f, 0.f};
#pragma unroll
        for (int k = 0; k < SW; ++k) {
            const float w = win.w[k];
#pragma unroll
            for (int o = 0; o < 4; ++o) a[o] = fmaf(w, X[o + k], a[o]);
        }
        *reinterpret_cast<float4*>(&hz[m][r][q]) = make_float4(a[0], a[1], a[2], a[3]);
    }
    __syncthreads();
    if (tid < 128) {
        const int r0 = (tid >> 4) * 2, col = tid & 15;
        const int px = bx * ST + col;
        float g[3][2];
#pragma unroll
        for (int m = 0; m < 3; ++m) {
            float v[12];
#pragma unroll
            for (int k = 0; k < 12; ++k) v[k] = hz[m][r0 + k][col];
#pragma unroll
            for (int o = 0; o < 2; ++o) {
                float acc = 0.f;
#pragma unroll
                for (int k = 0; k < SW; ++k) acc = fmaf(win.w[k], v[o + k], acc);
                g[m][o] = acc;
            }
        }
#pragma unroll
        for (int o = 0; o < 2; ++o) {
            const int py = by * ST + r0 + o;
            if (px < W && py < H) {
                float out = 0.f;
                if (own_kb[o] != 0) {
                    const float x = own_x[o], y = own_y[o];
                    out = g[0][o] + 2.f * x * g[1][o] + y * g[2][o] + mse_scale * (x - y);
                }
                st_f32(d_render, (pixel_index(py, W, px)) * 4u + ch * plane_b, out);
            }
        }
    }
}

__global__ void __launch_bounds__(1024) loss_fold_kernel(const float* __restrict__ p_ssim, int n_ssim,
                                                         const float* __restrict__ p_grad, int n_grad,
                                                         float* __restrict__ sums) {
    float acc[5] = {0.f, 0.f, 0.f, 0.f, 0.f};
    for (int r = threadIdx.x; r < n_ssim; r += 1024) acc[1] += p_ssim[r];
    for (int r = threadIdx.x; r < n_grad; r += 1024) {
        const float4 q = reinterpret_cast<const float4*>(p_grad)[r];
        acc[0] += q.x; acc[2] += q.y; acc[3] += q.z; acc[4] += q.w;
    }
    __shared__ float red[16][5];
#pragma unroll
    for (int q = 0; q < 5; ++q) {
        const float s = wave_sum_to_lane63(acc[q]);
        if ((threadIdx.x & 63) == 63) red[threadIdx.x >> 6][q] = s;
    }
    __syncthreads();
    if (threadIdx.x < 8) {
        float t = 0.f;
        if (threadIdx.x < 5)
            for (int w = 0; w < 16; ++w) t += red[w][threadIdx.x];
        sums[threadIdx.x] = t;
    }
}

static Win make_window() {
    Win w;
    float s = 0.f;
    for (int i = 0; i < SW; ++i) {
        const double d = (double)(i - SR);
        w.w[i] = (float)exp(-(d * d) / (2.0 * 1.5 * 1.5));
        s += w.w[i];
    }
    for (int i = 0; i < SW; ++i) w.w[i] /= s;
    return w;
}

}

using namespace gfl;

extern "C" {

static inline size_t align_up256(size_t v) { return (v + 255) / 256 * 256; }

size_t gfl_loss_workspace_bytes(int W, int H) {
    if (W <= 0 || H <= 0) return 0;
    const size_t gx = (W + ST - 1) / ST, gy = (H + ST - 1) / ST;
    return align_up256((size_t)9 * W * H * sizeof(float)) + align_up256(gx * gy * 3 * sizeof(float)) +
           align_up256(gx * gy * 4 * sizeof(float));
}

static int loss_launch(const float* render, const float* gt_rgb, const float* gt_depth, const uint8_t* keep,
                       const float* depth_ab, float lambda_rgb, float lambda_depth, int W, int H, float* d_render,
                       float* err_px, float* sums, void* workspace, size_t workspace_bytes, gfl_stream_t stream,
                       const float** p_ssim_out, int* n_ssim, const float** p_grad_out, int* n_grad,
                       const float* gt_stats = nullptr) {
    if (W <= 0 || H <= 0 || !render || !gt_rgb || !d_render || !err_px || !workspace) return GFL_ERR_INVALID;
    if (lambda_depth != 0.f && (!gt_depth || !depth_ab)) return GFL_ERR_INVALID;
    if (workspace_bytes < gfl_loss_workspace_bytes(W, H)) return GFL_ERR_WORKSPACE;
    if ((uint64_t)W * (uint64_t)H * 36u >= (1ull << 32) || W >= (1 << 24) || H >= (1 << 24))
        return GFL_ERR_INVALID;
    hipStream_t s = (hipStream_t)stream;
    const int gx = (W + ST - 1) / ST, gy = (H + ST - 1) / ST;
    float* dmaps = (float*)workspace;
    float* p_ssim = (float*)((char*)workspace + align_up256((size_t)9 * W * H * sizeof(float)));
    float* p_grad = (float*)((char*)p_ssim + align_up256((size_t)gx * gy * 3 * sizeof(float)));
    static const Win win = make_window();
    const float hw = (float)W * (float)H;
    const float s_scale = -lambda_rgb / (3.f * hw);
    float* st = const_cast<float*>(gt_stats);
    auto stats = gt_stats ? (keep ? ssim_stats_kernel<1, true> : ssim_stats_kernel<1, false>)
                          : (keep ? ssim_stats_kernel<0, true> : ssim_stats_kernel<0, false>);
    stats<<<gx * gy * 3, 256, 0, s>>>(render, gt_rgb, keep, W, H, gx, gy, win, s_scale, dmaps, p_ssim, st);
    auto grad = keep ? loss_grad_kernel<true> : loss_grad_kernel<false>;
    grad<<<gx * gy * 4, 256, 0, s>>>(render, gt_rgb, gt_depth, keep, depth_ab, dmaps, W, H, gx, gy, win,
                                     lambda_rgb * 2.f / (3.f * hw), lambda_depth / hw, d_render, err_px, p_grad);
    if (sums) loss_fold_kernel<<<1, 1024, 0, s>>>(p_ssim, gx * gy * 3, p_grad, gx * gy, sums);
    if (p_ssim_out) { *p_ssim_out = p_ssim; *n_ssim = gx * gy * 3; *p_grad_out = p_grad; *n_grad = gx * gy; }
    return check_launch();
}

int gfl_loss_fwd_bwd(const float* render, const float* gt_rgb, const float* gt_depth, const uint8_t* keep,
                     const float* depth_ab, float lambda_rgb, float lambda_depth, int W, int H, float* d_render,
                     float* err_px, float* sums, void* workspace, size_t workspace_bytes, gfl_stream_t stream) {
    if (!sums) return GFL_ERR_INVALID;
    return loss_launch(render, gt_rgb, gt_depth, keep, depth_ab, lambda_rgb, lambda_depth, W, H, d_render, err_px, sums,
                       workspace, workspace_bytes, stream, nullptr, nullptr, nullptr, nullptr);
}

int gfl_loss_fwd_bwd_partials(const float* render, const float* gt_rgb, const float* gt_depth, const uint8_t* keep,
                              const float* depth_ab, float lambda_rgb, float lambda_depth, int W, int H,
                              float* d_render, float* err_px, void* workspace, size_t workspace_bytes,
                              const float** p_ssim, int* n_ssim, const float** p_grad, int* n_grad,
                              gfl_stream_t stream) {
    if (!p_ssim || !n_ssim || !p_grad || !n_grad) return GFL_ERR_INVALID;
    return loss_launch(render, gt_rgb, gt_depth, keep, depth_ab, lambda_rgb, lambda_depth, W, H, d_render, err_px,
                       nullptr, workspace, workspace_bytes, stream, p_ssim, n_ssim, p_grad, n_grad);
}

int gfl_loss_prepare_gt(const float* gt_rgb, const uint8_t* keep, int W, int H, float* gt_stats, gfl_stream_t stream) {
    if (W <= 0 || H <= 0 || !gt_rgb || !gt_stats) return GFL_ERR_INVALID;
    if ((uint64_t)W * (uint64_t)H * 36u >= (1ull << 32) || W >= (1 << 24) || H >= (1 << 24)) return GFL_ERR_INVALID;
    const int gx = (W + ST - 1) / ST, gy = (H + ST - 1) / ST;
    static const Win win = make_window();
    auto stats = keep ? ssim_stats_kernel<2, true> : ssim_stats_kernel<2, false>;
    stats<<<gx * gy * 3, 256, 0, (hipStream_t)stream>>>(nullptr, gt_rgb, keep, W, H, gx, gy, win, 0.f, nullptr, nullptr,
                                                        gt_stats);
    return check_launch();
}

int gfl_loss_fwd_bwd_partials_cached(const float* render, const float* gt_rgb, const float* gt_depth,
                                     const uint8_t* keep, const float* depth_ab, float lambda_rgb, float lambda_depth,
                                     int W, int H, float* d_render, float* err_px, void* workspace,
                                     size_t workspace_bytes, const float* gt_stats, const float** p_ssim, int* n_ssim,
                                     const float** p_grad, int* n_grad, gfl_stream_t stream) {
    if (!p_ssim || !n_ssim || !p_grad || !n_grad) return GFL_ERR_INVALID;
    return loss_launch(render, gt_rgb, gt_depth, keep, depth_ab, lambda_rgb, lambda_depth, W, H, d_render, err_px,
                       nullptr, workspace, workspace_bytes, stream, p_ssim, n_ssim, p_grad, n_grad, gt_stats);
}

}
```

gflow_amd/fused.py:

```python
import ctypes

import torch

from . import _lib as L

ROW = 16
REC = 12
COLS = {"xyz": (0, 3), "scale": (3, 6), "rotate": (6, 10), "opacity": (10, 11), "rgb": (11, 14)}

_P = ctypes.c_void_p
_I = ctypes.c_int32


class FitState(ctypes.Structure):
    _fields_ = [("N", _I), ("cap", _I), ("W", _I), ("H", _I), ("K_cap", _I), ("gt_cached", _I),
                ("params", _P), ("adam_m", _P), ("adam_v", _P), ("rec", _P), ("d_rec", _P),
                ("flow_target", _P), ("flow_w", _P), ("still_target", _P), ("still_w", _P), ("row_flags", _P),
                ("pose", _P), ("pose_m", _P), ("pose_v", _P),
                ("depth_ab", _P), ("depth_ab_m", _P), ("depth_ab_v", _P),
                ("intr", _P), ("extr", _P), ("d_extr", _P), ("step", _P),
                ("gt_rgb", _P), ("gt_depth", _P), ("keep", _P), ("move_mask", _P), ("foot_flags", _P),
                ("render", _P), ("final_T", _P), ("n_contrib", _P),
                ("d_render", _P), ("err_px", _P), ("sums", _P),
                ("tile_offsets", _P), ("ids", _P), ("tile_range", _P), ("overflow", _P),
                ("workspace", _P), ("workspace_bytes", ctypes.c_size_t), ("cu_count", _I), ("flags", _I)]

GFL_FIT_DETERMINISTIC = 1


class FitHyper(ctypes.Structure):
    _fields_ = [("bg", ctypes.c_float), ("nearest", ctypes.c_float), ("extent", ctypes.c_float),
                ("lambda_rgb", ctypes.c_float), ("lambda_depth", ctypes.c_float), ("lambda_var", ctypes.c_float),
                ("lambda_flow", ctypes.c_float), ("lambda_still", ctypes.c_float), ("lambda_scale", ctypes.c_float),
                ("lr", ctypes.c_float), ("lr_camera", ctypes.c_float), ("beta1", ctypes.c_float),
                ("beta2", ctypes.c_float), ("eps", ctypes.c_float), ("lr_end_factor", ctypes.c_float),
                ("total_iters", _I), ("freeze_rgb", _I), ("freeze_all_splats", _I), ("step_camera", _I)]


def _declare(lib):
    if getattr(lib, "_fit_declared", False):
        return
    lib.gfl_fit_workspace_bytes.restype = ctypes.c_size_t
    lib.gfl_fit_workspace_bytes.argtypes = [ctypes.c_int] * 4
    for name in ("gfl_fit_forward", "gfl_fit_backward_step", "gfl_fit_iteration", "gfl_render_fwd"):
        fn = getattr(lib, name)
        fn.restype = ctypes.c_int
        fn.argtypes = [ctypes.POINTER(FitState), ctypes.POINTER(FitHyper), _P]
    lib.gfl_fit_iterations.restype = ctypes.c_int
    lib.gfl_fit_iterations.argtypes = [ctypes.POINTER(FitState), ctypes.POINTER(FitHyper), ctypes.c_int, ctypes.c_int, _P]
    lib.gfl_fit_snapshot.restype = ctypes.c_int
    lib.gfl_fit_snapshot.argtypes = [ctypes.POINTER(FitState), ctypes.POINTER(FitHyper), _P, _P, _P, ctypes.c_size_t, _P]
    lib.gfl_fit_iteration_snapshot.restype = ctypes.c_int
    lib.gfl_fit_iteration_snapshot.argtypes = [ctypes.POINTER(FitState), ctypes.POINTER(FitHyper), _P, _P, _P]
    lib.gfl_render_bwd.restype = ctypes.c_int
    lib.gfl_render_bwd.argtypes = [ctypes.POINTER(FitState), ctypes.POINTER(FitHyper), _P, _P, _P, _P, _P, _P]
    lib._fit_declared = True


PROFILE = {"mask": 0}

import gc as _gc
import threading as _threading

_GRAPH_LOCK = _threading.RLock()


def set_profile(mask):
    PROFILE["mask"] = int(mask)
    L.check(L.load().gfl_profile_enable(int(mask)), "profile")


class FitEngine:
    def __init__(self, W, H, capacity, device, K_cap=None, bg=0.0, cu_count=0, deterministic=False):
        self.lib = L.load()
        self.cu_count = int(cu_count)
        self._deterministic = bool(deterministic)
        _declare(self.lib)
        self.dev = torch.device(device)
        if self.dev.type != "cuda":
            raise RuntimeError("FitEngine needs a HIP device (there is no CPU path)")
        self.W, self.H = int(W), int(H)
        self.gx, self.gy = (self.W + 15) // 16, (self.H + 15) // 16
        self.T = self.gx * self.gy
        self.N = 0
        self.hp = FitHyper(bg=bg, nearest=0.2, extent=1.3, lambda_rgb=1.0, lambda_depth=0.0, lambda_var=0.0,
                           lambda_flow=0.0, lambda_still=0.0, lambda_scale=0.0, lr=1e-2, lr_camera=0.0, beta1=0.9, beta2=0.999,
                           eps=1e-8, lr_end_factor=0.1, total_iters=0, freeze_rgb=0, freeze_all_splats=0,
                           step_camera=1)
        f32 = dict(dtype=torch.float32, device=self.dev)
        i32 = dict(dtype=torch.int32, device=self.dev)
        H_, W_ = self.H, self.W
        self.pose = torch.zeros(7, **f32)
        self.pose[3:4].fill_(1.0)
        self.pose_m, self.pose_v = torch.zeros(7, **f32), torch.zeros(7, **f32)
        self.depth_ab = torch.zeros(2, **f32)
        self.depth_ab[0:1].fill_(1.0)
        self.ab_m, self.ab_v = torch.zeros(2, **f32), torch.zeros(2, **f32)
        self.intr = torch.zeros(4, **f32)
        self.extr = torch.zeros(12, **f32)
        self.d_extr = torch.zeros(12, **f32)
        self.step = torch.zeros(1, **i32)
        self.render = torch.zeros(4, H_, W_, **f32)
        self.final_T = torch.zeros(H_, W_, **f32)
        self.n_contrib = torch.zeros(H_, W_, **i32)
        self.d_render = torch.zeros(4, H_, W_, **f32)
        self.err_px = torch.zeros(H_, W_, **f32)
        self.sums = torch.zeros(8, **f32)
        self._offsets_and_flags = torch.zeros(self.T + 1 + 4, **i32)
        self.tile_offsets = self._offsets_and_flags[:self.T + 1]
        self.tile_range = torch.zeros(self.T, 2, **i32)
        self.overflow = self._offsets_and_flags[self.T + 1:]
        self.gt_rgb = self.gt_depth = self.keep = None
        self.move_mask = self.foot_flags = None
        self.flow_target = self.flow_w = self.still_target = self.still_w = self.row_flags = None
        self.cap = self.K_cap = 0
        self.K_cap_req = K_cap
        self._K_grown = False
        self.params = self.d_rec = self._state = None
        self.want_d_rec = False
        self._graphs, self._graph_key, self._graph_trash = {}, None, []
        self._reserved_sup = (None, 0)
        self.regions_outgrown = self.pairs_grown = 0
        self._pend_event = self._pend_host = self._ovf_event = self._ovf_host = None
        self._snap_ring = self._snap_ring_done = None
        self._snap_out = self._snap_ws = self._capture_stream = None
        self._launched = False
        self._reserved_N = -1
        self.busy = False
        self._alloc(int(capacity))

    def __del__(self):
        try:
            with _GRAPH_LOCK:
                self._graphs.clear()
                for gs in getattr(self, "_graph_trash", []):
                    gs.clear()
        except Exception:
            pass

    def _retire_graphs(self):
        if self._graphs:
            self._graph_trash.append(self._graphs)
            self._graphs = {}
        if len(self._graph_trash) > 256:
            self.reap_graphs()

    def reap_graphs(self):
        if self._graph_trash:
            with _GRAPH_LOCK:
                for gs in self._graph_trash:
                    gs.clear()
            self._graph_trash = []

    def _alloc(self, cap):
        f32 = dict(dtype=torch.float32, device=self.dev)
        old = self.params
        n = self.N
        self.cap = cap
        self.params = torch.zeros(cap, ROW, **f32)
        self.adam_m = torch.zeros(cap, ROW, **f32)
        self.adam_v = torch.zeros(cap, ROW, **f32)
        self.rec = torch.zeros(cap, REC, **f32)
        self.d_rec = torch.zeros(cap, REC, **f32) if self.want_d_rec else None
        if old is not None and n:
            self.params[:n] = old[:n]
        k_min = self.K_cap if self._K_grown else 0
        self._alloc_pairs(max(int(self.K_cap_req) if self.K_cap_req else max(4_000_000, 8 * cap), k_min))

    def _alloc_pairs(self, K_cap):
        self.K_cap = int(K_cap)
        self.ids = torch.zeros(self.K_cap, dtype=torch.int32, device=self.dev)
        nbytes = self.lib.gfl_fit_workspace_bytes(self.cap, self.K_cap, self.W, self.H)
        self.workspace = torch.zeros(nbytes, dtype=torch.uint8, device=self.dev)
        self._state = None
        self._reserved_N = -1

    def ensure_capacity(self, n):
        if n > self.cap:
            regs = (self.flow_target, self.flow_w, self.still_target, self.still_w, self.row_flags, self.foot_flags)
            m, v = self.adam_m, self.adam_v
            old_n = self.N
            self._alloc(max(n, 2 * self.cap))
            self.adam_m[:old_n], self.adam_v[:old_n] = m[:old_n], v[:old_n]
            grown = []
            for t in regs:
                if t is None:
                    grown.append(None)
                    continue
                g = torch.zeros((self.cap,) + tuple(t.shape[1:]), dtype=t.dtype, device=self.dev)
                g[:t.shape[0]] = t
                grown.append(g)
            self.flow_target, self.flow_w, self.still_target, self.still_w, self.row_flags, self.foot_flags = grown

    def set_count(self, n):
        if n > self.cap:
            raise RuntimeError("FitEngine.set_count beyond the capacity; call ensure_capacity first")
        self.N = int(n)
        if self._state is not None:
            self._state.N = self.N
        self._reserved_N = -1

    def invalidate_regions(self):
        self._reserved_N = -1

    def set_splats(self, attrs):
        n = attrs["xyz"].shape[0]
        self.ensure_capacity(n)
        self.N = n
        for k, (a, b) in COLS.items():
            self.params[:n, a:b] = attrs[k].detach().reshape(n, b - a).to(self.dev)
        self.params[:n, 14:] = 0
        self._state = None
        self._reserved_N = -1

    def views(self):
        return {k: self.params[:self.N, a:b] for k, (a, b) in COLS.items()}

    def reset_optimizer(self, splats=True, camera=True):
        if splats:
            self.adam_m.zero_()
            self.adam_v.zero_()
        if camera:
            self.pose_m.zero_(); self.pose_v.zero_(); self.ab_m.zero_(); self.ab_v.zero_()
        self.step.zero_()

    def set_targets(self, gt_image, gt_depth=None, keep=None):
        self.gt_rgb = gt_image.to(self.dev).float().contiguous()
        self.gt_depth = None if gt_depth is None else gt_depth.to(self.dev).float().reshape(self.H, self.W).contiguous()
        self.keep = None if keep is None else keep.to(self.dev).reshape(self.H, self.W).to(torch.uint8).contiguous()
        self.move_mask = self.foot_flags = None
        self._state = None

    def set_footprint_mask(self, move_mask, moving_rows):
        self.move_mask = move_mask.to(self.dev).reshape(self.H, self.W).to(torch.uint8).contiguous()
        flags = torch.zeros(self.cap, dtype=torch.uint8, device=self.dev)
        flags[:moving_rows.shape[0]] = moving_rows.to(self.dev).to(torch.uint8)
        self.foot_flags = flags
        if self.hp.bg > 0.0:
            self.keep = torch.zeros(self.H, self.W, dtype=torch.uint8, device=self.dev)
        else:
            self.keep = (self.move_mask == 0).to(torch.uint8).contiguous()
        self._state = None

    def set_regularisers(self, flow_target=None, flow_w=None, still_target=None, still_w=None, row_flags=None):
        def pad(t, width, dtype):
            if t is None:
                return None
            out = torch.zeros((self.cap, width) if width else (self.cap,), dtype=dtype, device=self.dev)
            out[:t.shape[0]] = t.to(self.dev).reshape((t.shape[0], width) if width else (t.shape[0],))
            return out
        self.flow_target, self.flow_w = pad(flow_target, 2, torch.float32), pad(flow_w, 0, torch.float32)
        self.still_target, self.still_w = pad(still_target, 3, torch.float32), pad(still_w, 0, torch.float32)
        self.row_flags = pad(row_flags, 0, torch.uint8)
        self._state = None

    def state(self):
        if self._state is None:
            s = FitState()
            s.N, s.cap, s.W, s.H, s.K_cap = self.N, self.cap, self.W, self.H, self.K_cap
            for name, ctype in FitState._fields_:
                if ctype is _P:
                    t = getattr(self, {"depth_ab_m": "ab_m", "depth_ab_v": "ab_v"}.get(name, name))
                    setattr(s, name, None if t is None else t.data_ptr())
            s.workspace_bytes = self.workspace.numel()
            s.cu_count = self.cu_count
            s.flags = GFL_FIT_DETERMINISTIC if self._deterministic else 0
            if self.gt_rgb is not None and self.foot_flags is None:
                L.check(self.lib.gfl_fit_prepare_targets(ctypes.byref(s), L.stream()), "fit prepare targets")
                s.gt_cached = 1
            self._state = s
        return self._state

    @property
    def deterministic(self):
        return self._deterministic

    @deterministic.setter
    def deterministic(self, on):
        self._deterministic = bool(on)
        if self._state is not None:
            self._state.flags = GFL_FIT_DETERMINISTIC if self._deterministic else 0

    def snapshot_ring(self, rows):
        ring = self._snap_ring
        if ring is None or ring.shape[0] < rows:
            ring = torch.empty(int(rows), 3, self.H, self.W, 3, dtype=torch.uint8, device=self.dev)
            self._snap_ring = ring
        if self._snap_ring_done is not None:
            torch.cuda.current_stream().wait_event(self._snap_ring_done)
        return ring[:rows]

    def snapshot_ring_copied(self):
        self._snap_ring_done = torch.cuda.Event()
        self._snap_ring_done.record()

    def forward(self):
        L.check(self.lib.gfl_fit_forward(ctypes.byref(self.state()), ctypes.byref(self.hp), L.stream()), "fit forward")

    def backward_step(self):
        L.check(self.lib.gfl_fit_backward_step(ctypes.byref(self.state()), ctypes.byref(self.hp), L.stream()),
                "fit backward/step")
        self._reserved_N = self.N

    GFL_ITER_RESERVED = 8

    def _reserved_flag(self):
        if self._reserved_N != self.N or self.N <= 0:
            return 0
        key = (self.W, self.H, self.K_cap)
        if self._reserved_sup[0] != key:
            self._reserved_sup = (key, int(self.lib.gfl_fit_reserved_supported(ctypes.byref(self.state()),
                                                                                ctypes.byref(self.hp))))
        return self.GFL_ITER_RESERVED if self._reserved_sup[1] else 0

    def iteration(self, use_graph=False, count=1, snapshot=False, flags=0, reserved=None):
        if snapshot:
            from .color import lut
            assert count == 1
            if self._snap_out is None:
                self._snap_out = torch.empty(3, self.H, self.W, 3, dtype=torch.uint8, device=self.dev)
            snap_args = (L.ptr(lut("turbo", self.dev)), L.ptr(self._snap_out))
        reserved = 0 if (flags or reserved is False or snapshot) else self._reserved_flag()
        gkey = ("snap", count, reserved) if snapshot else (count, reserved)
        if use_graph and not PROFILE["mask"] and self._launched and not flags:
            key = bytes(self.state()) + bytes(self.hp)
            if self._graph_key != key:
                self._retire_graphs()
                self._graph_key = key
            g = self._graphs.get(gkey)
            if g is None:
                if self._capture_stream is None:
                    self._capture_stream = torch.cuda.Stream(device=self.dev)
                side = self._capture_stream
                cur = torch.cuda.current_stream()
                st, hp = self.state(), self.hp
                with _GRAPH_LOCK:
                    gc_on = _gc.isenabled()
                    _gc.disable()
                    try:
                        g = torch.cuda.CUDAGraph()
                        side.wait_stream(cur)
                        with torch.cuda.stream(side):
                            g.capture_begin(capture_error_mode="thread_local")
                            try:
                                if snapshot:
                                    L.check(self.lib.gfl_fit_iteration_snapshot(ctypes.byref(st), ctypes.byref(hp), *snap_args,
                                                                                L.stream()), "snapshot iteration (capture)")
                                else:
                                    L.check(self.lib.gfl_fit_iterations(ctypes.byref(st), ctypes.byref(hp), count, reserved,
                                                                        L.stream()), "fit iterations (capture)")
                            finally:
                                g.capture_end()
                        cur.wait_stream(side)
                    finally:
                        if gc_on:
                            _gc.enable()
                self._graphs[gkey] = g
            g.replay()
            self._reserved_N = self.N
            return self._snap_out if snapshot else None
        if snapshot:
            L.check(self.lib.gfl_fit_iteration_snapshot(ctypes.byref(self.state()), ctypes.byref(self.hp), *snap_args, L.stream()),
                    "snapshot iteration")
        else:
            L.check(self.lib.gfl_fit_iterations(ctypes.byref(self.state()), ctypes.byref(self.hp), count, int(flags) | reserved,
                                                L.stream()), "fit iterations")
        self._reserved_N = self.N
        self._launched = True
        return self._snap_out if snapshot else None

    def snapshot(self, out=None):
        from .color import lut
        need = self.lib.gfl_fit_snapshot_workspace_bytes(self.N, self.W, self.H)
        if self._snap_ws is None or self._snap_ws.numel() < need:
            self._snap_ws = torch.empty(int(need * 1.5), dtype=torch.uint8, device=self.dev)
        if out is None:
            out = torch.empty(3, self.H, self.W, 3, dtype=torch.uint8, device=self.dev)
        L.check(self.lib.gfl_fit_snapshot(ctypes.byref(self.state()), ctypes.byref(self.hp), L.ptr(lut("turbo", self.dev)),
                                          L.ptr(out), L.ptr(self._snap_ws), self._snap_ws.numel(), L.stream()), "snapshot")
        return out

    _STATE_TENSORS = ("step", "pose", "pose_m", "pose_v", "depth_ab", "ab_m", "ab_v")

    def save_state(self):
        n = self.N
        out = {"N": n, "rows": [t[:n].clone() for t in (self.params, self.adam_m, self.adam_v)]}
        for k in self._STATE_TENSORS:
            out[k] = getattr(self, k).clone()
        return out

    def restore_state(self, saved):
        n = saved["N"]
        if n != self.N:
            raise RuntimeError("FitEngine.restore_state: the splat count has changed since save_state")
        self._reserved_N = -1
        for dst, src in zip((self.params, self.adam_m, self.adam_v), saved["rows"]):
            torch.bitwise_or(src.view(torch.int32), 0, out=dst[:n].view(torch.int32))
        for k in self._STATE_TENSORS:
            t = getattr(self, k)
            torch.bitwise_or(saved[k].view(torch.int32), 0, out=t.view(torch.int32))

    @property
    def uv(self):
        return self.rec[:self.N, 0:2]

    @property
    def depth(self):
        return self.rec[:self.N, 9:10]

    @property
    def K(self):
        return int(self.tile_offsets[self.T].item())

    def schedule(self, forward=False):
        nq, cap = ctypes.c_int(), ctypes.c_int()
        lists, counts = ctypes.c_void_p(), ctypes.c_void_p()
        fn = self.lib.gfl_fit_schedule_info_fwd if forward else self.lib.gfl_fit_schedule_info
        L.check(fn(ctypes.byref(self.state()), ctypes.byref(nq), ctypes.byref(cap),
                   ctypes.byref(lists), ctypes.byref(counts)), "fit schedule info")
        off_l = lists.value - self.workspace.data_ptr()
        off_c = counts.value - self.workspace.data_ptr()
        torch.cuda.synchronize(self.dev)
        lst = self.workspace[off_l:off_l + 4 * nq.value * cap.value].view(torch.int32).reshape(nq.value, cap.value).cpu()
        cnt = self.workspace[off_c:off_c + 4 * nq.value].view(torch.int32).cpu()
        return [(lst[c, :int(cnt[c])] & 0xffff).long() for c in range(nq.value)]

    def check_overflow(self):
        self._ovf_event = None
        code = int(self.overflow[0].item())
        self.reap_graphs()
        if code:
            self.overflow.zero_()
            raise RuntimeError(self._overflow_message(code))

    def settle_overflow(self):
        self._ovf_event = None
        self._pend_event = None
        code, skipped = (int(v) for v in self.overflow[:2].tolist())
        self.reap_graphs()
        if code == 0:
            if skipped > 0:
                self._count_void(skipped)
            return max(skipped, 0)
        if code != 1:
            self.overflow.zero_()
            raise RuntimeError(self._overflow_message(code))
        self._double_pairs()
        self.overflow.zero_()
        return max(skipped, 0)

    def _count_void(self, skipped):
        self.overflow[1:2].zero_()
        self.regions_outgrown += skipped

    def _double_pairs(self):
        self._K_grown = True
        self._alloc_pairs(2 * self.K_cap)
        with _GRAPH_LOCK:
            self._graphs.clear()
        self._graph_key = None
        self.pairs_grown += 1

    def grow_pairs(self):
        self._pend_event = None
        self._double_pairs()

    def _overflow_message(self, code):
        if code == 2:
            return ("FitEngine: an iteration was told that the previous one had run its preprocess / reserved its tile regions, "
                    "and it had not")
        return f"FitEngine: more than K_cap={self.K_cap} splat-tile pairs; raise K_cap"

    def watch_pending(self):
        if self._pend_host is None:
            self._pend_host = torch.zeros(8, dtype=torch.int32, pin_memory=True)
        self._pend_host[0:5].copy_(self._offsets_and_flags[self.T:self.T + 5], non_blocking=True)
        self._pend_event = torch.cuda.Event()
        self._pend_event.record()

    def pending_ready(self):
        return self._pend_event is None or self._pend_event.query()

    def read_pending(self):
        if self._pend_event is None:
            return None
        self._pend_event.synchronize()
        self._pend_event = None
        v = self._pend_host.tolist()
        return v[1], v[2], v[0]

    def drop_pending(self):
        self._pend_event = None

    def take_pending(self):
        got = self.read_pending()
        if got is None:
            return None
        code, skipped, pairs = got
        if code != 0 or 2 * pairs > self.K_cap:
            if code == 0:
                torch.cuda.current_stream().synchronize()
                self.grow_pairs()
            return -1
        if skipped > 0:
            self._count_void(skipped)
        return max(skipped, 0)

    def watch_overflow(self):
        self.poll_overflow()
        if self._ovf_host is None:
            self._ovf_host = torch.zeros(1, dtype=torch.int32, pin_memory=True)
        self._ovf_host.copy_(self.overflow[0:1], non_blocking=True)
        self._ovf_event = torch.cuda.Event()
        self._ovf_event.record()

    def poll_overflow(self):
        ev = self._ovf_event
        if ev is not None and ev.query():
            self._ovf_event = None
            if int(self._ovf_host[0]):
                self.overflow.zero_()
                raise RuntimeError(self._overflow_message(int(self._ovf_host[0])))

    def loss_terms(self):
        hw = float(self.H * self.W)
        return self.sums[0] / hw + (1.0 - self.sums[1] / (3.0 * hw)), self.sums[2] / hw
```

include/gflow_hip.h:

```cpp
#ifndef GFLOW_HIP_H
#define GFLOW_HIP_H

#include <stddef.h>
#include <stdint.h>

#ifdef __cplusplus
extern "C" {
#endif

typedef void* gfl_stream_t;

typedef enum gfl_status {
    GFL_OK = 0,
    GFL_ERR_INVALID = -1,
    GFL_ERR_WORKSPACE = -2,
    GFL_ERR_HIP = -3
} gfl_status;

#define GFL_TILE 16
#ifndef GFL_NEAREST
#define GFL_NEAREST 0.2f
#endif
#ifndef GFL_EXTENT
#define GFL_EXTENT 1.3f
#endif
#ifndef GFL_FOV_CLAMP
#define GFL_FOV_CLAMP 1.3f
#endif
#ifndef GFL_LOWPASS
#define GFL_LOWPASS 0.3f
#endif
#ifndef GFL_EIG_FLOOR
#define GFL_EIG_FLOOR 0.1f
#endif
#ifndef GFL_RADIUS_SIGMA
#define GFL_RADIUS_SIGMA 3.0f
#endif
#ifndef GFL_ALPHA_MIN
#define GFL_ALPHA_MIN (1.0f / 255.0f)
#endif
#ifndef GFL_ALPHA_MAX
#define GFL_ALPHA_MAX 0.99f
#endif
#ifndef GFL_T_MIN
#define GFL_T_MIN 1e-4f
#endif
#ifndef GFL_PIXEL_CENTER
#define GFL_PIXEL_CENTER 0.0f
#endif
#define GFL_MAX_BLEND_CHANNELS 4

#define GFL_VERSION 308
int gfl_version(void);
int gfl_constants(float* out10);
#define GFL_N_CONSTANTS 11
int gfl_constants_n(float* out, int n);
int gfl_ewa_on_mfma(void);
const char* gfl_status_string(int status);
int gfl_last_hip_error(void);
size_t gfl_reduce_workspace_bytes(int N);

int gfl_project_point_fwd(const float* xyz, const float* intr, const float* extr, int N, int W, int H,
                          float nearest, float extent, float* uv, float* depth, gfl_stream_t stream);
int gfl_project_point_bwd(const float* xyz, const float* intr, const float* extr, const float* depth,
                          const float* d_uv, const float* d_depth, int N, float* d_xyz, float* d_extr,
                          void* workspace, size_t workspace_bytes, gfl_stream_t stream);

int gfl_cov3d_fwd(const float* scale, const float* rotate, const uint8_t* visible, int N, float* cov3d,
                  gfl_stream_t stream);
int gfl_cov3d_bwd(const float* scale, const float* rotate, const uint8_t* visible, const float* d_cov3d,
                  int N, float* d_scale, float* d_rotate, gfl_stream_t stream);

int gfl_ewa_fwd(const float* xyz, const float* cov3d, const float* intr, const float* extr, const float* uv,
                const uint8_t* visible, int N, int W, int H, float* conic, int32_t* radius,
                int32_t* tiles_touched, gfl_stream_t stream);
int gfl_ewa_bwd(const float* xyz, const float* cov3d, const float* intr, const float* extr,
                const int32_t* radius, const float* d_conic, int N, int W, int H, float* d_xyz,
                float* d_cov3d, float* d_extr, void* workspace, size_t workspace_bytes, gfl_stream_t stream);

size_t gfl_bin_workspace_bytes(int N, int K_cap, int W, int H);
int gfl_bin_count(const float* uv, const int32_t* radius, const float* cutoff, int N, int W, int H,
                  int32_t* tile_offsets, gfl_stream_t stream);
int gfl_bin_sort(const float* uv, const float* depth, const int32_t* radius, const float* cutoff, int N, int W,
                 int H, const int32_t* tile_offsets, int K_cap, int32_t* ids, int32_t* tile_range,
                 int32_t* overflow, void* workspace, size_t workspace_bytes, gfl_stream_t stream);

int gfl_blend_fwd(const float* uv, const float* conic, const float* opacity, const float* feature,
                  int C_total, int c0, int C, const int32_t* ids, const int32_t* tile_range, float bg, int W,
                  int H, float* out, float* final_T, int32_t* n_contrib, gfl_stream_t stream);
int gfl_blend_bwd(const float* uv, const float* conic, const float* opacity, const float* feature,
                  int C_total, int c0, int C, const int32_t* ids, const int32_t* tile_range, float bg, int W,
                  int H, const float* final_T, const int32_t* n_contrib, const float* d_out, int N,
                  float* d_uv, float* d_conic, float* d_opacity, float* d_feature, int zero_first,
                  gfl_stream_t stream);

int gfl_sh_fwd(const float* shs, const float* dirs, const uint8_t* visible, int N, int K, float* out,
               gfl_stream_t stream);
int gfl_sh_bwd(const float* shs, const float* dirs, const uint8_t* visible, const float* d_out, int N, int K,
               float* d_shs, float* d_dirs, gfl_stream_t stream);

int gfl_colormap_nonzero(const float* value, int N, const float* lut, float* out, void* workspace,
                         size_t workspace_bytes, gfl_stream_t stream);

size_t gfl_loss_workspace_bytes(int W, int H);
int gfl_loss_fwd_bwd_partials(const float* render, const float* gt_rgb, const float* gt_depth, const uint8_t* keep,
                              const float* depth_ab, float lambda_rgb, float lambda_depth, int W, int H,
                              float* d_render, float* err_px, void* workspace, size_t workspace_bytes,
                              const float** p_ssim, int* n_ssim, const float** p_grad, int* n_grad,
                              gfl_stream_t stream);
int gfl_loss_prepare_gt(const float* gt_rgb, const uint8_t* keep, int W, int H, float* gt_stats, gfl_stream_t stream);
int gfl_loss_fwd_bwd_partials_cached(const float* render, const float* gt_rgb, const float* gt_depth,
                                     const uint8_t* keep, const float* depth_ab, float lambda_rgb, float lambda_depth,
                                     int W, int H, float* d_render, float* err_px, void* workspace,
                                     size_t workspace_bytes, const float* gt_stats, const float** p_ssim, int* n_ssim,
                                     const float** p_grad, int* n_grad, gfl_stream_t stream);
int gfl_loss_fwd_bwd(const float* render, const float* gt_rgb, const float* gt_depth, const uint8_t* keep,
                     const float* depth_ab, float lambda_rgb, float lambda_depth, int W, int H,
                     float* d_render, float* err_px, float* sums, void* workspace, size_t workspace_bytes,
                     gfl_stream_t stream);

int gfl_adam_step(float* param, const float* grad, float* m, float* v, int64_t n, int row_len,
                  const uint8_t* row_zero_grad, float lr, float beta1, float beta2, float eps,
                  const int32_t* d_step, float lr_end_factor, int total_iters, gfl_stream_t stream);
int gfl_step_increment(int32_t* d_step, gfl_stream_t stream);

typedef struct gfl_fit_state {
    int32_t N, cap, W, H, K_cap;
    int32_t gt_cached;
    float *params, *adam_m, *adam_v;
    float *rec, *d_rec;
    const float *flow_target, *flow_w, *still_target, *still_w;
    const uint8_t* row_flags;
    float *pose, *pose_m, *pose_v;
    float *depth_ab, *depth_ab_m, *depth_ab_v;
    const float* intr;
    float* extr;
    float* d_extr;
    int32_t* step;
    const float* gt_rgb;
    const float* gt_depth;
    uint8_t* keep;
    const uint8_t* move_mask;
    const uint8_t* foot_flags;
    float *render, *final_T;
    int32_t* n_contrib;
    float *d_render, *err_px, *sums;
    int32_t *tile_offsets, *ids, *tile_range, *overflow;
    void* workspace;
    size_t workspace_bytes;
    int32_t cu_count;
    int32_t flags;
} gfl_fit_state;

#define GFL_FIT_DETERMINISTIC 1

typedef struct gfl_fit_hyper {
    float bg, nearest, extent;
    float lambda_rgb, lambda_depth, lambda_var, lambda_flow, lambda_still;
    float lambda_scale;
    float lr, lr_camera, beta1, beta2, eps, lr_end_factor;
    int32_t total_iters;
    int32_t freeze_rgb;
    int32_t freeze_all_splats;
    int32_t step_camera;
} gfl_fit_hyper;

size_t gfl_fit_workspace_bytes(int cap, int K_cap, int W, int H);
int gfl_fit_forward(const gfl_fit_state* st, const gfl_fit_hyper* hp, gfl_stream_t stream);
int gfl_fit_backward_step(const gfl_fit_state* st, const gfl_fit_hyper* hp, gfl_stream_t stream);
int gfl_fit_iteration(const gfl_fit_state* st, const gfl_fit_hyper* hp, gfl_stream_t stream);
#define GFL_ITER_RESERVED 8
int gfl_fit_iterations(const gfl_fit_state* st, const gfl_fit_hyper* hp, int count, int flags, gfl_stream_t stream);
int gfl_fit_reserved_supported(const gfl_fit_state* st, const gfl_fit_hyper* hp);
int gfl_render_fwd(const gfl_fit_state* st, const gfl_fit_hyper* hp, gfl_stream_t stream);
int gfl_render_bwd(const gfl_fit_state* st, const gfl_fit_hyper* hp, const float* d_render, const float* d_uv,
                   const float* d_depth, float* d_params, float* d_extr, gfl_stream_t stream);
size_t gfl_fit_snapshot_workspace_bytes(int N, int W, int H);
int gfl_fit_snapshot(const gfl_fit_state* st, const gfl_fit_hyper* hp, const float* lut, uint8_t* out_u8, void* workspace,
                     size_t workspace_bytes, gfl_stream_t stream);
int gfl_fit_iteration_snapshot(const gfl_fit_state* st, const gfl_fit_hyper* hp, const float* lut, uint8_t* out_u8,
                               gfl_stream_t stream);
int gfl_fit_snapshot_stage(const gfl_fit_state* src, const gfl_fit_state* dst, gfl_stream_t stream);
int gfl_fit_prepare_targets(const gfl_fit_state* st, gfl_stream_t stream);
int gfl_fit_schedule_info(const gfl_fit_state* st, int* n_queues, int* queue_capacity, const int32_t** d_lists,
                          const int32_t** d_counts);
int gfl_fit_schedule_info_fwd(const gfl_fit_state* st, int* n_queues, int* queue_capacity, const int32_t** d_lists,
                              const int32_t** d_counts);
int gfl_tile_sort_only(const int32_t* tile_offsets, int T, int K_cap, void* keys, int32_t* ids,
                       int32_t* tile_range, gfl_stream_t stream);
#define GFL_SORT_MAX_SPLIT 64
#define GFL_SORT_ORDER_TRAILER (GFL_SORT_MAX_SPLIT + 4)
int gfl_tile_sort_ordered(const int32_t* order, int W, int H, int K_cap, void* keys, int32_t* ids, int32_t* tile_range,
                          gfl_stream_t stream);
int gfl_tile_sort_reserved(const int32_t* order, const int32_t* fill, int32_t* tile_counts, int32_t* void_words, int W, int H,
                           int K_cap, void* keys, int32_t* ids, int32_t* tile_range, gfl_stream_t stream);

int gfl_selftest_reduce10(const float* in, float* out_scatter, float* out_dpp, gfl_stream_t stream);
int gfl_selftest_cov2d(const float* m, const float* cov, int n, float* out_valu, float* out_mfma, gfl_stream_t stream);
int gfl_selftest_block_mask(const float* rec, int n, int x0, int y0, int box, int32_t* mask, int32_t* truth, gfl_stream_t stream);

int gfl_concave_hull(const double* points_xy, int n, double concavity, double length_threshold, double* ring_xy,
                     int cap_vertices);

#define GFL_SCAN_CHUNK 2048
size_t gfl_scan_f64_workspace_bytes(int n);
int gfl_scan_f64(const double* in, int n, double* out, void* workspace, size_t workspace_bytes, gfl_stream_t stream);

size_t gfl_track_anchor_workspace_bytes(int n_new, int N);
int gfl_track_anchor(const float* uv, int uv_stride, int N, const double* query_xy, int n_new, int32_t* anchor,
                     double* shift_xy, void* workspace, size_t workspace_bytes, gfl_stream_t stream);
int gfl_track_frame(const float* uv, int uv_stride, const float* depth, int depth_stride, int N, const float* depth_map,
                    int W, int H, const int32_t* anchor, const double* shift_xy, int n_anchored, int frame, int T,
                    float occ_threshold, float* tracks, uint8_t* occluded, gfl_stream_t stream);

int gfl_seg_score(const uint8_t* pred, const uint8_t* gt, const uint8_t* valid, int T, int H, int W, int radius,
                  uint32_t* counts, gfl_stream_t stream);

size_t gfl_recon_workspace_bytes(int W, int H);
int gfl_recon_frame(const float* render, const float* gt_rgb, int W, int H, int frame, int T, double* sums, void* workspace,
                    size_t workspace_bytes, gfl_stream_t stream);

int gfl_abi_sizes(int* sizeof_fit_state, int* sizeof_fit_hyper);

#define GFL_PROFILE_STAGES 9
int gfl_profile_enable(unsigned stage_mask);
int gfl_profile_read(double* total_ms, int* counts, int n_stages);

#ifdef __cplusplus
}
#endif
#endif
```

Baseline: 10.49.

## Fuse SSIM loss-gradient adjoint into blend backward prologue

By default the separate loss_grad kernel launch goes away. The stats kernel gets a fourth block slice per tile that handles the depth term. The SSIM adjoint convolution for the RGB d_render gradient now runs in the prologue of the fused blend-backward kernel, using LDS that overlays the walk buffers. This removes one full-image launch plus the write-then-read of d_render for RGB. In exchange it adds LDS and register pressure to the blend-backward kernel and requires the Gaussian window to match a hardcoded literal. The old path is kept behind a flag.

```diff
diff --git a/gflow_amd/_lib.py b/gflow_amd/_lib.py
--- a/gflow_amd/_lib.py
+++ b/gflow_amd/_lib.py
@@ -14,7 +14,7 @@
 
 c_void_p, c_int, c_float, c_size_t, c_int64 = ctypes.c_void_p, ctypes.c_int, ctypes.c_float, ctypes.c_size_t, ctypes.c_int64
 
-MIN_VERSION = 308
+MIN_VERSION = 309
 
 _P = c_void_p
 SIGNATURES = {
diff --git a/gflow_amd/csrc/gfl_fit.hip b/gflow_amd/csrc/gfl_fit.hip
--- a/gflow_amd/csrc/gfl_fit.hip
+++ b/gflow_amd/csrc/gfl_fit.hip
@@ -189,7 +189,7 @@
 static int fit_check(const gfl_fit_state* st, const gfl_fit_hyper* hp) {
     if (!st || !hp) return GFL_ERR_INVALID;
     if (st->N < 0 || st->N > st->cap || st->W <= 0 || st->H <= 0 || st->K_cap < 0) return GFL_ERR_INVALID;
-    if (st->flags & ~GFL_FIT_DETERMINISTIC) return GFL_ERR_INVALID;
+    if (st->flags & ~(GFL_FIT_DETERMINISTIC | GFL_FIT_LOSS_GRAD_LAUNCH)) return GFL_ERR_INVALID;
     if (!st->params || !st->rec || !st->pose || !st->intr || !st->extr || !st->render || !st->final_T ||
         !st->n_contrib || !st->tile_offsets || !st->ids || !st->tile_range || !st->overflow || !st->workspace)
         return GFL_ERR_INVALID;
@@ -382,7 +382,7 @@
     {
         StageScope p(ST_BLEND_BWD, s);
         const TileQueue q = {w.sched.list, w.sched.count, w.sched.counters + w.sched.nq, w.sched.nq, w.sched.cap_q};
-        launch_blend_bwd(st, hp->bg, gx, gy, blend_grid(st, T), 10, d_render, q, w, LossTail{}, s);
+        launch_blend_bwd(st, hp->bg, gx, gy, blend_grid(st, T), 10, d_render, q, w, LossTail{}, nullptr, s);
     }
     {
         StageScope p(ST_PRE_BWD_ADAM, s);
@@ -403,13 +403,20 @@
     const FitWs w = carve(st);
     const float *p_ssim = nullptr, *p_grad = nullptr;
     int n_ssim = 0, n_grad = 0;
+    const bool grad_launch = (st->flags & GFL_FIT_LOSS_GRAD_LAUNCH) != 0;
+    AdjointArgs adj = {};
     {
         StageScope p(ST_LOSS, s);
         const float* gt_stats = (st->gt_cached && !st->foot_flags) ? w.gt_stats : nullptr;
-        rc = gfl_loss_fwd_bwd_partials_cached(st->render, st->gt_rgb, st->gt_depth, st->keep, st->depth_ab,
-                                              hp->lambda_rgb, hp->lambda_depth, st->W, st->H, st->d_render,
-                                              st->err_px, w.loss_ws, w.loss_ws_bytes, gt_stats, &p_ssim, &n_ssim,
-                                              &p_grad, &n_grad, stream);
+        if (grad_launch)
+            rc = gfl_loss_fwd_bwd_partials_cached(st->render, st->gt_rgb, st->gt_depth, st->keep, st->depth_ab,
+                                                  hp->lambda_rgb, hp->lambda_depth, st->W, st->H, st->d_render,
+                                                  st->err_px, w.loss_ws, w.loss_ws_bytes, gt_stats, &p_ssim, &n_ssim,
+                                                  &p_grad, &n_grad, stream);
+        else
+            rc = launch_loss_stats_depth(st->render, st->gt_rgb, st->gt_depth, st->keep, st->depth_ab, hp->lambda_rgb,
+                                         hp->lambda_depth, st->W, st->H, st->d_render, st->err_px, w.loss_ws, w.loss_ws_bytes,
+                                         gt_stats, &p_ssim, &n_ssim, &p_grad, &n_grad, &adj, s);
     }
     if (rc) return rc;
     AdamCfg ac = {hp->lr, hp->beta1, hp->beta2, hp->eps, hp->lr_end_factor, hp->total_iters};
@@ -428,7 +435,7 @@
         StageScope p(ST_BLEND_BWD, s);
         const TileQueue q = {w.sched.list, w.sched.count, w.sched.counters + w.sched.nq, w.sched.nq, w.sched.cap_q};
         const int sums = hp->freeze_all_splats ? 6 : (hp->freeze_rgb ? 7 : 10);
-        launch_blend_bwd(st, hp->bg, gx, gy, blend_grid(st, T), sums, st->d_render, q, w, lt, s);
+        launch_blend_bwd(st, hp->bg, gx, gy, blend_grid(st, T), sums, st->d_render, q, w, lt, grad_launch ? nullptr : &adj, s);
     }
     const int rows = reduce_rows(st->N > 0 ? st->N : 1);
     RegCfg rcfg;
diff --git a/gflow_amd/csrc/gfl_fit.hpp b/gflow_amd/csrc/gfl_fit.hpp
--- a/gflow_amd/csrc/gfl_fit.hpp
+++ b/gflow_amd/csrc/gfl_fit.hpp
@@ -1,4 +1,5 @@
 #pragma once
+#include "gfl_loss_adjoint.hpp"
 #include "gfl_math.hpp"
 #include "gfl_profile.hpp"
 #include "gfl_sched.hpp"
@@ -302,7 +303,11 @@
 void launch_snapshot_u8(const float* a, const float* b, const float* c, int P, uint8_t* out, hipStream_t s);
 void launch_snapshot_stage(const StageCopy& c, hipStream_t s);
 void launch_blend_bwd(const gfl_fit_state* st, float bg, int gx, int gy, int grid, int sums, const float* d_out, const TileQueue& q,
-                      const FitWs& w, const LossTail& lt, hipStream_t s);
+                      const FitWs& w, const LossTail& lt, const AdjointArgs* adj, hipStream_t s);
+int launch_loss_stats_depth(const float* render, const float* gt_rgb, const float* gt_depth, const uint8_t* keep,
+                            const float* depth_ab, float lambda_rgb, float lambda_depth, int W, int H, float* d_render,
+                            float* err_px, void* workspace, size_t workspace_bytes, const float* gt_stats, const float** p_ssim,
+                            int* n_ssim, const float** p_grad, int* n_grad, AdjointArgs* adjoint, hipStream_t stream);
 void launch_splat_bwd_adam(const gfl_fit_state* st, const FitWs& w, int gx, int gy, const RegCfg& rc, const AdamCfg& ac,
                            const NextSched& ns, int extra, size_t lds, hipStream_t s);
 void launch_splat_bwd_op(const gfl_fit_state* st, const FitWs& w, int gx, int gy, const NextSched& ns, int extra, size_t lds,
diff --git a/gflow_amd/csrc/gfl_fit_bwd.hip b/gflow_amd/csrc/gfl_fit_bwd.hip
--- a/gflow_amd/csrc/gfl_fit_bwd.hip
+++ b/gflow_amd/csrc/gfl_fit_bwd.hip
@@ -91,7 +91,7 @@
     }
 }
 
-template <int SUMS, bool DET = false>
+template <int SUMS, bool DET = false, bool ADJ = false>
 __global__ void __launch_bounds__(256, 8) fused_blend_bwd_kernel(const float* __restrict__ rec,
                                                               const int32_t* __restrict__ ids,
                                                               const int32_t* __restrict__ tile_range, float bg, int W,
@@ -103,25 +103,32 @@
                                                               const float* __restrict__ ckpt,
                                                               const float* __restrict__ render, LossTail ltail, int gy,
                                                               const int32_t* __restrict__ wide_off, long long wide_base,
-                                                              const int32_t* __restrict__ stamp_ptr) {
+                                                              const int32_t* __restrict__ stamp_ptr, AdjointArgs adj) {
     if (ltail.enabled && blockIdx.x == gridDim.x - queue.nq) loss_tail(ltail);
     constexpr int NB = DET ? FBB_DET : FBB;
     constexpr int NACC = DET ? 4 : 1;
     static_assert(!DET || NACC * NB * REC == 3 * 4 * 256, "the deterministic rows are cleared with three float4 per lane");
-    __shared__ RecLDS recs[NB];
-    __shared__ int32_t s_gid[NB];
-    __shared__ float acc[NACC][NB][REC];
-    __shared__ unsigned char s_mask[NB];
+    struct WalkLds {
+        RecLDS recs[NB];
+        float acc[NACC][NB][REC];
+        int32_t gid[NB];
+        unsigned char mask[NB];
+    };
+    static_assert(!ADJ || (size_t)ADJ_LDS_FLOATS * sizeof(float) <= sizeof(RecLDS) * NB + sizeof(float) * NACC * NB * REC,
+                  "the prologue's buffers overlay recs and acc");
+    __shared__ __attribute__((aligned(16))) WalkLds wl;
+    RecLDS (&recs)[NB] = wl.recs;
+    int32_t (&s_gid)[NB] = wl.gid;
+    float (&acc)[NACC][NB][REC] = wl.acc;
+    unsigned char (&s_mask)[NB] = wl.mask;
     __shared__ int32_t s_max_last;
     __shared__ int32_t s_ticket;
     __shared__ int32_t s_simd[4];
-    const int tid = threadIdx.x, wave = tid >> 6, lane = tid & 63;
-    const int comp_few = SUMS == 6 ? reduce_scatter6_component(lane) : reduce_scatter7_component(lane);
-    const int comp = SUMS == 10 ? reduce_scatter10_component(lane) : (comp_few == SUMS - 1 ? 9 : comp_few);
+    const int tid_k = threadIdx.x, wave = tid_k >> 6, lane_k = tid_k & 63;
     unsigned hw_id;
     asm volatile("s_getreg_b32 %0, hwreg(HW_REG_HW_ID)" : "=s"(hw_id));
     const int simd = (hw_id >> 4) & 3;
-    if (lane == 0) s_simd[wave] = simd;
+    if (lane_k == 0) s_simd[wave] = simd;
     __syncthreads();
     const bool simd_ok = ((1 << s_simd[0]) | (1 << s_simd[1]) | (1 << s_simd[2]) | (1 << s_simd[3])) == 15;
   for (bool first = true;; first = false) {
@@ -132,8 +139,8 @@
     const bool plan_ok = simd_ok && ((1 << (plan & 3)) | (1 << ((plan >> 2) & 3)) | (1 << ((plan >> 4) & 3)) | (1 << ((plan >> 6) & 3))) == 15;
     const int blk = plan_ok ? (int)((plan >> (2 * simd)) & 3u) : wave;
     const int tx = tile % gx, ty = tile / gx;
-    const int px = tx * GFL_TILE + (blk & 1) * 8 + (lane & 7);
-    const int py = ty * GFL_TILE + (blk >> 1) * 8 + (lane >> 3);
+    const int px = tx * GFL_TILE + (blk & 1) * 8 + (lane_k & 7);
+    const int py = ty * GFL_TILE + (blk >> 1) * 8 + (lane_k >> 3);
     const bool inside = px < W && py < H;
     const float fx = pixf(px), fy = pixf(py);
     const int start = tile_range[2 * tile], end = tile_range[2 * tile + 1];
@@ -150,12 +157,39 @@
 
     float g0 = 0.f, g1 = 0.f, g2 = 0.f, g3 = 0.f, T = 1.f, S = 0.f;
     int last = 0;
+    float T_far = 1.f;
+    if (ADJ) {
+        float g[3];
+        adjoint_tile(adj, render, reinterpret_cast<float*>(&wl), tx, ty, (blk & 1) * 8 + (lane_k & 7), (blk >> 1) * 8 + (lane_k >> 3),
+                     px, py, inside, W, H, g, [&] {
+                         if (inside) {
+                             const size_t pix = (size_t)py * W + px, plane = (size_t)H * W;
+                             last = n_contrib[pix];
+                             g3 = d_out[3 * plane + pix];
+                             if (last_part) T_far = final_T[pix];
+                         }
+                     });
+        g0 = g[0]; g1 = g[1]; g2 = g[2];
+        if (inside && last_part) {
+            const unsigned pb = pixel_index(py, W, px) * 4u, plane_b = (unsigned)H * (unsigned)W * 4u;
+            st_f32(adj.d_render, pb, g0);
+            st_f32(adj.d_render, pb + plane_b, g1);
+            st_f32(adj.d_render, pb + 2u * plane_b, g2);
+        }
+    }
+    int tid_w = tid_k;
+    if constexpr (ADJ) asm volatile("" : "+v"(tid_w));
+    const int tid = tid_w, lane = tid & 63;
+    const int comp_few = SUMS == 6 ? reduce_scatter6_component(lane) : reduce_scatter7_component(lane);
+    const int comp = SUMS == 10 ? reduce_scatter10_component(lane) : (comp_few == SUMS - 1 ? 9 : comp_few);
     if (inside) {
         const size_t pix = (size_t)py * W + px, plane = (size_t)H * W;
-        last = n_contrib[pix];
-        g0 = d_out[pix]; g1 = d_out[plane + pix]; g2 = d_out[2 * plane + pix]; g3 = d_out[3 * plane + pix];
+        if (!ADJ) {
+            last = n_contrib[pix];
+            g0 = d_out[pix]; g1 = d_out[plane + pix]; g2 = d_out[2 * plane + pix]; g3 = d_out[3 * plane + pix];
+        }
         if (last_part) {
-            T = final_T[pix];
+            T = ADJ ? T_far : final_T[pix];
             S = T * bg * (g0 + g1 + g2 + g3);
         } else {
             const float* ck = ckpt + ((size_t)item.queue * (HEAVY_PARTS - 1) + item.part) * 5 * 256 + blk * 64 + lane;
@@ -305,13 +339,20 @@
 }
 
 void launch_blend_bwd(const gfl_fit_state* st, float bg, int gx, int gy, int grid, int sums, const float* d_out, const TileQueue& q,
-                      const FitWs& w, const LossTail& lt, hipStream_t s) {
-    auto kern = sums == 6 ? fused_blend_bwd_kernel<6> : (sums == 7 ? fused_blend_bwd_kernel<7> : fused_blend_bwd_kernel<10>);
-    if (st->flags & GFL_FIT_DETERMINISTIC)
-        kern = sums == 6 ? fused_blend_bwd_kernel<6, true>
-                         : (sums == 7 ? fused_blend_bwd_kernel<7, true> : fused_blend_bwd_kernel<10, true>);
+                      const FitWs& w, const LossTail& lt, const AdjointArgs* adj, hipStream_t s) {
+    const bool det = (st->flags & GFL_FIT_DETERMINISTIC) != 0;
+    auto pick = [&](auto k6, auto k7, auto k10) { return sums == 6 ? k6 : (sums == 7 ? k7 : k10); };
+    auto kern = pick(fused_blend_bwd_kernel<6>, fused_blend_bwd_kernel<7>, fused_blend_bwd_kernel<10>);
+    if (det && adj)
+        kern = pick(fused_blend_bwd_kernel<6, true, true>, fused_blend_bwd_kernel<7, true, true>, fused_blend_bwd_kernel<10, true, true>);
+    else if (det)
+        kern = pick(fused_blend_bwd_kernel<6, true>, fused_blend_bwd_kernel<7, true>, fused_blend_bwd_kernel<10, true>);
+    else if (adj)
+        kern = pick(fused_blend_bwd_kernel<6, false, true>, fused_blend_bwd_kernel<7, false, true>,
+                    fused_blend_bwd_kernel<10, false, true>);
     kern<<<grid, 256, 0, s>>>(st->rec, st->ids, st->tile_range, bg, st->W, st->H, gx, st->final_T, st->n_contrib, d_out, w.pair_grad,
-                              q, w.sched.work, w.ckpt, st->render, lt, gy, w.wide_off, w.wide_base, w.stamp);
+                              q, w.sched.work, w.ckpt, st->render, lt, gy, w.wide_off, w.wide_base, w.stamp,
+                              adj ? *adj : AdjointArgs{});
 }
 
 #ifdef GFL_TRACE
diff --git a/gflow_amd/csrc/gfl_loss_adjoint.hpp b/gflow_amd/csrc/gfl_loss_adjoint.hpp
--- /dev/null
+++ b/gflow_amd/csrc/gfl_loss_adjoint.hpp
@@ -0,0 +1,245 @@
+#pragma once
+#include "gfl_common.hpp"
+
+#include <math.h>
+#include <string.h>
+
+namespace gfl {
+
+constexpr int SW = 11;
+constexpr int SR = SW / 2;
+constexpr int ST = 16;
+constexpr int SI = ST + 2 * SR;
+
+struct Win { float w[SW]; };
+
+inline Win make_window() {
+    Win w;
+    float s = 0.f;
+    for (int i = 0; i < SW; ++i) {
+        const double d = (double)(i - SR);
+        w.w[i] = (float)exp(-(d * d) / (2.0 * 1.5 * 1.5));
+        s += w.w[i];
+    }
+    for (int i = 0; i < SW; ++i) w.w[i] /= s;
+    return w;
+}
+
+struct WinLiteral {
+    __host__ __device__ constexpr float operator[](int k) const {
+        constexpr float w[SW] = {0x1.0d956ep-10f, 0x1.f1fe04p-8f, 0x1.26eb18p-5f, 0x1.bff1p-4f, 0x1.b43c4p-3f, 0x1.106562p-2f,
+                                 0x1.b43c4p-3f, 0x1.bff1p-4f, 0x1.26eb18p-5f, 0x1.f1fe04p-8f, 0x1.0d956ep-10f};
+        return w[k];
+    }
+};
+inline bool window_is_literal(const Win& win) {
+    for (int k = 0; k < SW; ++k) {
+        const float lit = WinLiteral{}[k];
+        if (memcmp(&lit, &win.w[k], sizeof(float)) != 0) return false;
+    }
+    return true;
+}
+
+__device__ __forceinline__ void load16(const float* __restrict__ row, float (&v)[16]) {
+    const float4* p = reinterpret_cast<const float4*>(row);
+    const float4 a = p[0], b = p[1], c = p[2], d = p[3];
+    v[0] = a.x; v[1] = a.y; v[2] = a.z; v[3] = a.w; v[4] = b.x; v[5] = b.y; v[6] = b.z; v[7] = b.w;
+    v[8] = c.x; v[9] = c.y; v[10] = c.z; v[11] = c.w; v[12] = d.x; v[13] = d.y; v[14] = d.z; v[15] = d.w;
+}
+
+__device__ __forceinline__ float ld_f32(const float* __restrict__ base, unsigned byte_off) {
+    return *reinterpret_cast<const float*>(reinterpret_cast<const char*>(base) + byte_off);
+}
+__device__ __forceinline__ unsigned pixel_index(int y, int W, int x) { return __umul24((unsigned)y, (unsigned)W) + (unsigned)x; }
+__device__ __forceinline__ void st_f32(float* __restrict__ base, unsigned byte_off, float v) {
+    *reinterpret_cast<float*>(reinterpret_cast<char*>(base) + byte_off) = v;
+}
+
+template <class Weights>
+__device__ __forceinline__ void adjoint_row4(const float* __restrict__ src, const Weights& wt, float* __restrict__ dst) {
+#pragma clang fp contract(off)
+    float X[16];
+    load16(src, X);
+    float a[4] = {0.f, 0.f, 0.f, 0.f};
+#pragma unroll
+    for (int k = 0; k < SW; ++k) {
+        const float w = wt[k];
+#pragma unroll
+        for (int o = 0; o < 4; ++o) a[o] = __builtin_fmaf(w, X[o + k], a[o]);
+    }
+    *reinterpret_cast<float4*>(dst) = make_float4(a[0], a[1], a[2], a[3]);
+}
+
+template <class Weights>
+__device__ __forceinline__ float adjoint_col(const float* v, const Weights& wt) {
+#pragma clang fp contract(off)
+    float acc = 0.f;
+#pragma unroll
+    for (int k = 0; k < SW; ++k) acc = __builtin_fmaf(wt[k], v[k], acc);
+    return acc;
+}
+
+__device__ __forceinline__ float adjoint_combine(float c_mu1, float c_e11, float c_e12, float x, float y, float mse_scale) {
+#pragma clang fp contract(off)
+    const float t1 = (2.f * x) * c_e11, t2 = y * c_e12;
+    return __builtin_fmaf(mse_scale, x - y, (c_mu1 + t1) + t2);
+}
+
+struct DepthBlock {
+    const float* gt_depth;
+    const float* depth_ab;
+    float depth_scale;
+    float* d_render;
+    float* err_px;
+    float* partial;
+};
+
+template <bool KEEP>
+__device__ __forceinline__ void loss_depth_block(const float* __restrict__ render, const float* __restrict__ gt_rgb,
+                                                 const uint8_t* __restrict__ keep, const DepthBlock& db, int W, int H,
+                                                 int bx, int by, int tile) {
+#pragma clang fp contract(off)
+    const int tid = threadIdx.x;
+    const size_t plane = (size_t)H * W;
+    const int lx = tid & 15, ly = tid >> 4;
+    const int px = bx * ST + lx, py = by * ST + ly;
+    float v[4] = {0.f, 0.f, 0.f, 0.f};
+    if (px < W && py < H) {
+        const size_t pix = (size_t)py * W + px;
+        const int kb = KEEP ? (int)keep[pix] : 1;
+        float rr[3], gg[3];
+#pragma unroll
+        for (int c = 0; c < 3; ++c) {
+            rr[c] = render[c * plane + pix];
+            gg[c] = gt_rgb[pix * 3 + c];
+        }
+        const bool with_depth = db.depth_scale != 0.f;
+        const float D = with_depth ? render[3 * plane + pix] : 0.f;
+        const float gt = with_depth ? db.gt_depth[pix] : 0.f;
+        const bool k = kb != 0;
+        float e = 0.f;
+#pragma unroll
+        for (int c = 0; c < 3; ++c) {
+            const float d = k ? (rr[c] - gg[c]) : 0.f;
+            e = __builtin_fmaf(d, d, e);
+        }
+        e *= (1.f / 3.f);
+        db.err_px[pix] = e;
+        v[0] = e;
+        float gD = 0.f;
+        if (with_depth) {
+            const float a = db.depth_ab[0], b = db.depth_ab[1];
+            const float d = __builtin_fmaf(a, D, b);
+            const float diff = d - gt, sum = d + gt;
+            if (k) {
+                v[1] = diff * diff / sum;
+                const float dl = db.depth_scale * diff * (d + 3.f * gt) / (sum * sum);
+                gD = dl * a;
+                v[2] = dl * D;
+                v[3] = dl;
+            }
+        }
+        db.d_render[3 * plane + pix] = gD;
+    }
+    __shared__ float red[4][4];
+#pragma unroll
+    for (int q = 0; q < 4; ++q) {
+        const float s = wave_sum_to_lane63(v[q]);
+        if ((tid & 63) == 63) red[tid >> 6][q] = s;
+    }
+    __syncthreads();
+    if (tid < 4) db.partial[(size_t)tile * 4 + tid] = red[0][tid] + red[1][tid] + red[2][tid] + red[3][tid];
+}
+
+struct AdjointArgs {
+    const float* dmaps;
+    const float* gt_rgb;
+    const uint8_t* keep;
+    float mse_scale;
+    float* d_render;
+};
+
+#ifndef GFL_ADJ_MAPS
+#define GFL_ADJ_MAPS 3
+#endif
+constexpr int ADJ_MAPS = GFL_ADJ_MAPS;
+static_assert(ADJ_MAPS == 1 || ADJ_MAPS == 3, "GFL_ADJ_MAPS: 1 or 3");
+constexpr int ADJ_SP = ADJ_MAPS == 3 ? 32 : 48;
+constexpr int ADJ_HP = ADJ_MAPS == 3 ? 16 : 24;
+constexpr int ADJ_LDS_FLOATS = ADJ_MAPS * ((SI + 1) * ADJ_SP + SI * ADJ_HP);
+
+template <class Tail>
+__device__ __forceinline__ void adjoint_tile(const AdjointArgs& a, const float* __restrict__ render, float* lds, int tx,
+                                             int ty, int lc, int lr, int px, int py, bool inside, int W, int H,
+                                             float (&g)[3], Tail&& tail) {
+    float* const sm = lds;
+    float* const hz = lds + ADJ_MAPS * (SI + 1) * ADJ_SP;
+    int tid = threadIdx.x;
+    asm volatile("" : "+v"(tid));
+    const unsigned plane_b = (unsigned)H * (unsigned)W * 4u;
+    const int x0 = tx * ST - SR, y0 = ty * ST - SR;
+    const unsigned own_pix = inside ? pixel_index(py, W, px) : 0u;
+    int own_kb = 0;
+    if (inside) own_kb = a.keep ? (int)a.keep[own_pix] : 1;
+    constexpr int NG = 4;
+    const int sq = tid & 31, srg = tid >> 5;
+    const int sx = x0 + sq;
+    const bool in_x = sq < SI && sx >= 0 && sx < W;
+    unsigned pb[NG];
+    bool in[NG];
+#pragma unroll
+    for (int j = 0; j < NG; ++j) {
+        const int y = y0 + srg + 8 * j;
+        in[j] = in_x && (srg + 8 * j) < SI && (unsigned)y < (unsigned)H;
+        pb[j] = in[j] ? (pixel_index(y, W, sx)) << 2 : 0u;
+    }
+    float dm[NG][3];
+#pragma unroll
+    for (int j = 0; j < NG; ++j)
+#pragma unroll
+        for (int m = 0; m < 3; ++m) dm[j][m] = ld_f32(a.dmaps, pb[j] + (unsigned)m * plane_b);
+#pragma unroll
+    for (int ch = 0; ch < 3; ++ch) {
+        float conv[3];
+#pragma unroll
+        for (int m0 = 0; m0 < 3; m0 += ADJ_MAPS) {
+#pragma unroll
+            for (int j = 0; j < NG; ++j) {
+                const int r = min(srg + 8 * j, SI);
+#pragma unroll
+                for (int m = 0; m < ADJ_MAPS; ++m) sm[(m * (SI + 1) + r) * ADJ_SP + sq] = in[j] ? dm[j][m0 + m] : 0.f;
+            }
+            __syncthreads();
+            for (int it = tid; it < ADJ_MAPS * SI * 4; it += 256) {
+                const int m = it / (SI * 4), rem = it - m * (SI * 4);
+                const int r = rem >> 2, q = (rem & 3) * 4;
+                adjoint_row4(&sm[(m * (SI + 1) + r) * ADJ_SP + q], WinLiteral{}, &hz[(m * SI + r) * ADJ_HP + q]);
+            }
+            float own_x = 0.f, own_y = 0.f;
+            if (m0 + ADJ_MAPS == 3) {
+                own_x = ld_f32(render, own_pix * 4u + (unsigned)ch * plane_b);
+                own_y = ld_f32(a.gt_rgb, own_pix * 12u + (unsigned)ch * 4u);
+            }
+            if (m0 + ADJ_MAPS == 3 && ch == 2) tail();
+            if (m0 + ADJ_MAPS == 3 && ch < 2) {
+#pragma unroll
+                for (int j = 0; j < NG; ++j)
+#pragma unroll
+                    for (int m = 0; m < 3; ++m) dm[j][m] = ld_f32(a.dmaps, pb[j] + (unsigned)(3 * (ch + 1) + m) * plane_b);
+            }
+            __syncthreads();
+#pragma unroll
+            for (int m = 0; m < ADJ_MAPS; ++m) {
+                float v[SW];
+#pragma unroll
+                for (int k = 0; k < SW; ++k) v[k] = hz[(m * SI + lr + k) * ADJ_HP + lc];
+                conv[m0 + m] = adjoint_col(v, WinLiteral{});
+                asm volatile("" : "+v"(conv[m0 + m]));
+            }
+            if (m0 + ADJ_MAPS == 3)
+                g[ch] = own_kb != 0 ? adjoint_combine(conv[0], conv[1], conv[2], own_x, own_y, a.mse_scale) : 0.f;
+        }
+    }
+}
+
+}
diff --git a/gflow_amd/csrc/gfl_ssim.hip b/gflow_amd/csrc/gfl_ssim.hip
--- a/gflow_amd/csrc/gfl_ssim.hip
+++ b/gflow_amd/csrc/gfl_ssim.hip
@@ -1,34 +1,11 @@
-#include "gfl_common.hpp"
-
-#include <math.h>
+#include "gfl_loss_adjoint.hpp"
 
 namespace gfl {
 
-constexpr int SW = 11;
-constexpr int SR = SW / 2;
-constexpr int ST = 16;
-constexpr int SI = ST + 2 * SR;
 constexpr int SP = 48;
 constexpr int HP = 24;
 constexpr float SSIM_C1 = 0.01f * 0.01f;
 constexpr float SSIM_C2 = 0.03f * 0.03f;
-
-struct Win { float w[SW]; };
-
-__device__ __forceinline__ void load16(const float* __restrict__ row, float (&v)[16]) {
-    const float4* p = reinterpret_cast<const float4*>(row);
-    const float4 a = p[0], b = p[1], c = p[2], d = p[3];
-    v[0] = a.x; v[1] = a.y; v[2] = a.z; v[3] = a.w; v[4] = b.x; v[5] = b.y; v[6] = b.z; v[7] = b.w;
-    v[8] = c.x; v[9] = c.y; v[10] = c.z; v[11] = c.w; v[12] = d.x; v[13] = d.y; v[14] = d.z; v[15] = d.w;
-}
-
-__device__ __forceinline__ float ld_f32(const float* __restrict__ base, unsigned byte_off) {
-    return *reinterpret_cast<const float*>(reinterpret_cast<const char*>(base) + byte_off);
-}
-__device__ __forceinline__ unsigned pixel_index(int y, int W, int x) { return __umul24((unsigned)y, (unsigned)W) + (unsigned)x; }
-__device__ __forceinline__ void st_f32(float* __restrict__ base, unsigned byte_off, float v) {
-    *reinterpret_cast<float*>(reinterpret_cast<char*>(base) + byte_off) = v;
-}
 
 __device__ __forceinline__ void load12(const float* __restrict__ row, float (&v)[12]) {
     const float4* p = reinterpret_cast<const float4*>(row);
@@ -45,7 +22,7 @@
                                                          const uint8_t* __restrict__ keep, int W, int H, int gx,
                                                          int gy, Win win, float scale ,
                                                          float* __restrict__ dmaps, float* __restrict__ partial,
-                                                         float* __restrict__ gt_stats) {
+                                                         float* __restrict__ gt_stats, int per_tile, DepthBlock db) {
     constexpr int APITCH = 48, ROWS = SI + 1;
     __shared__ __attribute__((aligned(16))) v2f s_a[ROWS][APITCH];
     __shared__ __attribute__((aligned(16))) v2f s_b[MODE == 0 ? ROWS : 1][APITCH];
@@ -53,9 +30,13 @@
     __shared__ __attribute__((aligned(16))) v2f h_a[SI][ST];
     __shared__ __attribute__((aligned(16))) v2f h_b[MODE == 0 ? SI : 1][ST];
     __shared__ __attribute__((aligned(16))) float h_xy[MODE == 2 ? 1 : SI][ST];
-    const int lb = __builtin_amdgcn_readfirstlane(xcd_logical_block(blockIdx.x, gx * gy * 3));
-    const int c = lb % 3, tile = lb / 3;
+    const int lb = __builtin_amdgcn_readfirstlane(xcd_logical_block(blockIdx.x, gx * gy * per_tile));
+    const int c = per_tile == 4 ? (lb & 3) : lb % 3, tile = per_tile == 4 ? (lb >> 2) : lb / 3;
     const int bx = tile % gx, by = tile / gx;
+    if (MODE != 2 && c == 3) {
+        loss_depth_block<KEEP>(render, gt_rgb, keep, db, W, H, bx, by, tile);
+        return;
+    }
     const int x0 = bx * ST - SR, y0 = by * ST - SR;
     const int tid = threadIdx.x;
     const unsigned plane_b = (unsigned)H * (unsigned)W * 4u;
@@ -202,60 +183,13 @@
     __shared__ __attribute__((aligned(16))) float sm[3][SI + 1][SP];
     __shared__ __attribute__((aligned(16))) float hz[3][SI][HP];
     const int tid = threadIdx.x;
-    const size_t plane = (size_t)H * W;
     const unsigned plane_b = (unsigned)H * (unsigned)W * 4u;
     const int lb = __builtin_amdgcn_readfirstlane(xcd_logical_block(blockIdx.x, gx * gy * 4));
     const int ch = lb & 3, tile = lb >> 2;
     const int bx = tile % gx, by = tile / gx;
     if (ch == 3) {
-        const int lx = tid & 15, ly = tid >> 4;
-        const int px = bx * ST + lx, py = by * ST + ly;
-        float v[4] = {0.f, 0.f, 0.f, 0.f};
-        if (px < W && py < H) {
-            const size_t pix = (size_t)py * W + px;
-            const int kb = KEEP ? (int)keep[pix] : 1;
-            float rr[3], gg[3];
-#pragma unroll
-            for (int c = 0; c < 3; ++c) {
-                rr[c] = render[c * plane + pix];
-                gg[c] = gt_rgb[pix * 3 + c];
-            }
-            const bool with_depth = depth_scale != 0.f;
-            const float D = with_depth ? render[3 * plane + pix] : 0.f;
-            const float gt = with_depth ? gt_depth[pix] : 0.f;
-            const bool k = kb != 0;
-            float e = 0.f;
-#pragma unroll
-            for (int c = 0; c < 3; ++c) {
-                const float d = k ? (rr[c] - gg[c]) : 0.f;
-                e = fmaf(d, d, e);
-            }
-            e *= (1.f / 3.f);
-            err_px[pix] = e;
-            v[0] = e;
-            float gD = 0.f;
-            if (with_depth) {
-                const float a = depth_ab[0], b = depth_ab[1];
-                const float d = fmaf(a, D, b);
-                const float diff = d - gt, sum = d + gt;
-                if (k) {
-                    v[1] = diff * diff / sum;
-                    const float dl = depth_scale * diff * (d + 3.f * gt) / (sum * sum);
-                    gD = dl * a;
-                    v[2] = dl * D;
-                    v[3] = dl;
-                }
-            }
-            d_render[3 * plane + pix] = gD;
-        }
-        __shared__ float red[4][4];
-#pragma unroll
-        for (int q = 0; q < 4; ++q) {
-            const float s = wave_sum_to_lane63(v[q]);
-            if ((tid & 63) == 63) red[tid >> 6][q] = s;
-        }
-        __syncthreads();
-        if (tid < 4) partial[(size_t)tile * 4 + tid] = red[0][tid] + red[1][tid] + red[2][tid] + red[3][tid];
+        const DepthBlock db = {gt_depth, depth_ab, depth_scale, d_render, err_px, partial};
+        loss_depth_block<KEEP>(render, gt_rgb, keep, db, W, H, bx, by, tile);
         return;
     }
     const int x0 = bx * ST - SR, y0 = by * ST - SR;
@@ -303,16 +237,7 @@
     for (int it = tid; it < 3 * SI * 4; it += 256) {
         const int m = it / (SI * 4), rem = it - m * (SI * 4);
         const int r = rem >> 2, q = (rem & 3) * 4;
-        float X[16];
-        load16(&sm[m][r][q], X);
-        float a[4] = {0.f, 0.f, 0.f, 0.f};
-#pragma unroll
-        for (int k = 0; k < SW; ++k) {
-            const float w = win.w[k];
-#pragma unroll
-            for (int o = 0; o < 4; ++o) a[o] = fmaf(w, X[o + k], a[o]);
-        }
-        *reinterpret_cast<float4*>(&hz[m][r][q]) = make_float4(a[0], a[1], a[2], a[3]);
+        adjoint_row4(&sm[m][r][q], win.w, &hz[m][r][q]);
     }
     __syncthreads();
     if (tid < 128) {
@@ -325,12 +250,7 @@
 #pragma unroll
             for (int k = 0; k < 12; ++k) v[k] = hz[m][r0 + k][col];
 #pragma unroll
-            for (int o = 0; o < 2; ++o) {
-                float acc = 0.f;
-#pragma unroll
-                for (int k = 0; k < SW; ++k) acc = fmaf(win.w[k], v[o + k], acc);
-                g[m][o] = acc;
-            }
+            for (int o = 0; o < 2; ++o) g[m][o] = adjoint_col(v + o, win.w);
         }
 #pragma unroll
         for (int o = 0; o < 2; ++o) {
@@ -339,7 +259,7 @@
                 float out = 0.f;
                 if (own_kb[o] != 0) {
                     const float x = own_x[o], y = own_y[o];
-                    out = g[0][o] + 2.f * x * g[1][o] + y * g[2][o] + mse_scale * (x - y);
+                    out = adjoint_combine(g[0][o], g[1][o], g[2][o], x, y, mse_scale);
                 }
                 st_f32(d_render, (pixel_index(py, W, px)) * 4u + ch * plane_b, out);
             }
@@ -371,18 +291,6 @@
     }
 }
 
-static Win make_window() {
-    Win w;
-    float s = 0.f;
-    for (int i = 0; i < SW; ++i) {
-        const double d = (double)(i - SR);
-        w.w[i] = (float)exp(-(d * d) / (2.0 * 1.5 * 1.5));
-        s += w.w[i];
-    }
-    for (int i = 0; i < SW; ++i) w.w[i] /= s;
-    return w;
-}
-
 }
 
 using namespace gfl;
@@ -402,7 +310,7 @@
                        const float* depth_ab, float lambda_rgb, float lambda_depth, int W, int H, float* d_render,
                        float* err_px, float* sums, void* workspace, size_t workspace_bytes, gfl_stream_t stream,
                        const float** p_ssim_out, int* n_ssim, const float** p_grad_out, int* n_grad,
-                       const float* gt_stats = nullptr) {
+                       const float* gt_stats = nullptr, AdjointArgs* adjoint = nullptr) {
     if (W <= 0 || H <= 0 || !render || !gt_rgb || !d_render || !err_px || !workspace) return GFL_ERR_INVALID;
     if (lambda_depth != 0.f && (!gt_depth || !depth_ab)) return GFL_ERR_INVALID;
     if (workspace_bytes < gfl_loss_workspace_bytes(W, H)) return GFL_ERR_WORKSPACE;
@@ -419,10 +327,18 @@
     float* st = const_cast<float*>(gt_stats);
     auto stats = gt_stats ? (keep ? ssim_stats_kernel<1, true> : ssim_stats_kernel<1, false>)
                           : (keep ? ssim_stats_kernel<0, true> : ssim_stats_kernel<0, false>);
-    stats<<<gx * gy * 3, 256, 0, s>>>(render, gt_rgb, keep, W, H, gx, gy, win, s_scale, dmaps, p_ssim, st);
-    auto grad = keep ? loss_grad_kernel<true> : loss_grad_kernel<false>;
-    grad<<<gx * gy * 4, 256, 0, s>>>(render, gt_rgb, gt_depth, keep, depth_ab, dmaps, W, H, gx, gy, win,
-                                     lambda_rgb * 2.f / (3.f * hw), lambda_depth / hw, d_render, err_px, p_grad);
+    const float mse_scale = lambda_rgb * 2.f / (3.f * hw);
+    const DepthBlock db = {gt_depth, depth_ab, lambda_depth / hw, d_render, err_px, p_grad};
+    if (adjoint) {
+        if (!window_is_literal(win)) return GFL_ERR_INVALID;
+        stats<<<gx * gy * 4, 256, 0, s>>>(render, gt_rgb, keep, W, H, gx, gy, win, s_scale, dmaps, p_ssim, st, 4, db);
+        *adjoint = AdjointArgs{dmaps, gt_rgb, keep, mse_scale, d_render};
+    } else {
+        stats<<<gx * gy * 3, 256, 0, s>>>(render, gt_rgb, keep, W, H, gx, gy, win, s_scale, dmaps, p_ssim, st, 3, DepthBlock{});
+        auto grad = keep ? loss_grad_kernel<true> : loss_grad_kernel<false>;
+        grad<<<gx * gy * 4, 256, 0, s>>>(render, gt_rgb, gt_depth, keep, depth_ab, dmaps, W, H, gx, gy, win, mse_scale,
+                                         db.depth_scale, d_render, err_px, p_grad);
+    }
     if (sums) loss_fold_kernel<<<1, 1024, 0, s>>>(p_ssim, gx * gy * 3, p_grad, gx * gy, sums);
     if (p_ssim_out) { *p_ssim_out = p_ssim; *n_ssim = gx * gy * 3; *p_grad_out = p_grad; *n_grad = gx * gy; }
     return check_launch();
@@ -453,7 +369,7 @@
     static const Win win = make_window();
     auto stats = keep ? ssim_stats_kernel<2, true> : ssim_stats_kernel<2, false>;
     stats<<<gx * gy * 3, 256, 0, (hipStream_t)stream>>>(nullptr, gt_rgb, keep, W, H, gx, gy, win, 0.f, nullptr, nullptr,
-                                                        gt_stats);
+                                                        gt_stats, 3, DepthBlock{});
     return check_launch();
 }
 
@@ -468,3 +384,16 @@
 }
 
 }
+
+namespace gfl {
+
+int launch_loss_stats_depth(const float* render, const float* gt_rgb, const float* gt_depth, const uint8_t* keep,
+                            const float* depth_ab, float lambda_rgb, float lambda_depth, int W, int H, float* d_render,
+                            float* err_px, void* workspace, size_t workspace_bytes, const float* gt_stats, const float** p_ssim,
+                            int* n_ssim, const float** p_grad, int* n_grad, AdjointArgs* adjoint, hipStream_t stream) {
+    if (!p_ssim || !n_ssim || !p_grad || !n_grad || !adjoint) return GFL_ERR_INVALID;
+    return loss_launch(render, gt_rgb, gt_depth, keep, depth_ab, lambda_rgb, lambda_depth, W, H, d_render, err_px, nullptr,
+                       workspace, workspace_bytes, (gfl_stream_t)stream, p_ssim, n_ssim, p_grad, n_grad, gt_stats, adjoint);
+}
+
+}
diff --git a/gflow_amd/fused.py b/gflow_amd/fused.py
--- a/gflow_amd/fused.py
+++ b/gflow_amd/fused.py
@@ -26,6 +26,7 @@
                 ("workspace", _P), ("workspace_bytes", ctypes.c_size_t), ("cu_count", _I), ("flags", _I)]
 
 GFL_FIT_DETERMINISTIC = 1
+GFL_FIT_LOSS_GRAD_LAUNCH = 2
 
 
 class FitHyper(ctypes.Structure):
@@ -71,10 +72,11 @@
 
 
 class FitEngine:
-    def __init__(self, W, H, capacity, device, K_cap=None, bg=0.0, cu_count=0, deterministic=False):
+    def __init__(self, W, H, capacity, device, K_cap=None, bg=0.0, cu_count=0, deterministic=False, loss_grad_launch=False):
         self.lib = L.load()
         self.cu_count = int(cu_count)
         self._deterministic = bool(deterministic)
+        self._loss_grad_launch = bool(loss_grad_launch)
         _declare(self.lib)
         self.dev = torch.device(device)
         if self.dev.type != "cuda":
@@ -264,13 +266,26 @@
                     setattr(s, name, None if t is None else t.data_ptr())
             s.workspace_bytes = self.workspace.numel()
             s.cu_count = self.cu_count
-            s.flags = GFL_FIT_DETERMINISTIC if self._deterministic else 0
+            s.flags = self._flags()
             if self.gt_rgb is not None and self.foot_flags is None:
                 L.check(self.lib.gfl_fit_prepare_targets(ctypes.byref(s), L.stream()), "fit prepare targets")
                 s.gt_cached = 1
             self._state = s
         return self._state
 
+    def _flags(self):
+        return (GFL_FIT_DETERMINISTIC if self._deterministic else 0) | (GFL_FIT_LOSS_GRAD_LAUNCH if self._loss_grad_launch else 0)
+
+    @property
+    def loss_grad_launch(self):
+        return self._loss_grad_launch
+
+    @loss_grad_launch.setter
+    def loss_grad_launch(self, on):
+        self._loss_grad_launch = bool(on)
+        if self._state is not None:
+            self._state.flags = self._flags()
+
     @property
     def deterministic(self):
         return self._deterministic
@@ -279,7 +294,7 @@
     def deterministic(self, on):
         self._deterministic = bool(on)
         if self._state is not None:
-            self._state.flags = GFL_FIT_DETERMINISTIC if self._deterministic else 0
+            self._state.flags = self._flags()
 
     def snapshot_ring(self, rows):
         ring = self._snap_ring
diff --git a/include/gflow_hip.h b/include/gflow_hip.h
--- a/include/gflow_hip.h
+++ b/include/gflow_hip.h
@@ -50,7 +50,7 @@
 #endif
 #define GFL_MAX_BLEND_CHANNELS 4
 
-#define GFL_VERSION 308
+#define GFL_VERSION 309
 int gfl_version(void);
 int gfl_constants(float* out10);
 #define GFL_N_CONSTANTS 11
@@ -153,6 +153,7 @@
 } gfl_fit_state;
 
 #define GFL_FIT_DETERMINISTIC 1
+#define GFL_FIT_LOSS_GRAD_LAUNCH 2
 
 typedef struct gfl_fit_hyper {
     float bg, nearest, extent;
```

After: 9.917. -5.4%, worse.
